# fraunhoferhhi/vvenc

Hardware: AMD Instinct MI355X
Metric: frames/sec + bit-exact vs CPU, 1080p/4K 10-bit preset=faster at 1/2/4/8 GPU (higher is better)
Workload: dtype i16; 1 GPU; BASELINE configs[1]: hot-path work lists RECORDED from the reference encoder (1920x1080 10-bit synthetic clip, 65 frames, preset faster; one picture per temporal layer), replayed resident in HBM: a step = one picture's integer-ME SAD windows + sub-pel SATD stages + table calls + fused TU transform/quant lists + DMVR lists on 5 HIP streams; steps follow the GOP's 1:1:2:4:8:16 layer mix from the key; hip_streams=5, sample_pairs_per_frame=175309451, coefficients_per_frame=6951461, recorded_calls_outside_the_lists=0

## Files before the change

### include/vvenc_hip.h

```cpp
#ifndef VVENC_HIP_H
#define VVENC_HIP_H

#include <stddef.h>
#include <stdint.h>

#ifdef __cplusplus
extern "C" {
#endif

#define VVHIP_API __attribute__((visibility("default")))

enum {
  VVHIP_OK           = 0,
  VVHIP_E_ARG        = -1,
  VVHIP_E_HIP        = -2,
  VVHIP_E_NOMEM      = -3,
  VVHIP_E_UNSUPPORTED= -4
};

typedef struct vvhip_ctx vvhip_ctx;

VVHIP_API int         vvhip_create( vvhip_ctx** out, int device );
VVHIP_API void        vvhip_destroy( vvhip_ctx* ctx );
VVHIP_API const char* vvhip_last_error( const vvhip_ctx* ctx );
// ... 61 lines not shown
VVHIP_API int vvhip_planes_derive( vvhip_ctx* ctx, const int16_t* d_org_base, int org_stride, int org_rows, int16_t* d_org_tiled,
                                   const int16_t* d_cur_base, int cur_stride, int cur_rows, int16_t* d_cur_tiled, int16_t* d_cur_shift1 );
VVHIP_API size_t vvhip_tiled8_elems( int stride, int rows );
VVHIP_API int vvhip_plane_tile8( vvhip_ctx* ctx, const int16_t* d_base, int stride, int rows, int16_t* d_tiled );
VVHIP_API int vvhip_dist_multi_func_tiled( vvhip_ctx* ctx, const int16_t* d_org, int org_stride, const int16_t* d_cur, int cur_stride, const vvhip_tiled_planes* tiled_host, int bit_depth,
                                           const vvhip_dist_fjob* jobs_host, int n_jobs );

VVHIP_API int vvhip_sad_x5_batch( vvhip_ctx* ctx,
                                  const int16_t* d_org, int org_stride,
                                  const int16_t* d_cur, int cur_stride,
                                  int width, int height, int sub_shift, int calc_centre,
                                  const vvhip_dist_item* d_items, int n, uint64_t* d_out5 );

VVHIP_API int vvhip_sad_mask_batch( vvhip_ctx* ctx,
                                    const int16_t* d_org, int org_stride,
                                    const int16_t* d_cur, int cur_stride,
                                    const int16_t* d_mask, int mask_stride, int step_x, int mask_stride2,
                                    int width, int height, int sub_shift, int bit_depth,
                                    const vvhip_dist_item* d_items, const int32_t* d_mask_off, int n, uint64_t* d_out );

VVHIP_API int vvhip_fix_weighted_sse_batch( vvhip_ctx* ctx,
                                            const int16_t* d_org, int org_stride,
                                            const int16_t* d_cur, int cur_stride,
                                            int width, int height, int bit_depth,
                                            const vvhip_dist_item* d_items, const uint32_t* d_weights, int n, uint64_t* d_out );

VVHIP_API int vvhip_sad_surface( vvhip_ctx* ctx,
                                 const int16_t* d_org, int org_stride,
                                 const int16_t* d_ref, int ref_stride,
                                 int width, int height, int sub_shift,
                                 int range_x, int range_y,
                                 const int32_t* d_block_org_off, const int32_t* d_block_ref_off, int n_blocks,
                                 uint32_t* d_out );

enum { VVHIP_DCT2 = 0, VVHIP_DCT8 = 1, VVHIP_DST7 = 2 };

VVHIP_API int vvhip_fwd_transform_batch( vvhip_ctx* ctx, const int16_t* d_resi, int resi_stride, const int32_t* d_resi_off,
                                         int n, int width, int height, int tr_hor, int tr_ver, int bit_depth,
                                         int32_t* d_coef );
VVHIP_API int vvhip_inv_transform_batch( vvhip_ctx* ctx, const int32_t* d_coef,
                                         int n, int width, int height, int tr_hor, int tr_ver, int bit_depth,
                                         int16_t* d_resi, int resi_stride, const int32_t* d_resi_off );

typedef struct { int16_t qp; int16_t flags; } vvhip_tu_qp;

VVHIP_API int vvhip_quant_batch( vvhip_ctx* ctx, const int32_t* d_coef, int n, int width, int height, int bit_depth,
                                 const vvhip_tu_qp* d_qp, int thr_val,
                                 int16_t* d_level, int32_t* d_delta_u ,
                                 int32_t* d_abs_sum, int32_t* d_last_scan_pos );
VVHIP_API int vvhip_dequant_batch( vvhip_ctx* ctx, const int16_t* d_level, int n, int width, int height, int bit_depth,
                                   const vvhip_tu_qp* d_qp, int32_t* d_coef );
VVHIP_API int vvhip_need_rdoq_batch( vvhip_ctx* ctx, const int32_t* d_coef, int n, int width, int height, int bit_depth,
                                     const vvhip_tu_qp* d_qp, uint8_t* d_need );

VVHIP_API int vvhip_dequant_core( vvhip_ctx* ctx, int max_x, int max_y, int scale, const int16_t* d_level, size_t level_stride, int32_t* d_coef,
                                  int right_shift, int input_maximum, int32_t transform_maximum );
VVHIP_API int vvhip_quant_core( vvhip_ctx* ctx, const int32_t* d_coef, int width, int height, int quant_coeff, int q_bits, int64_t add, int thr_val,
                                int16_t* d_level , int32_t* d_delta_u , int32_t* d_abs_sum, int32_t* d_last_scan_pos );
VVHIP_API int vvhip_quant_core_lfnst( vvhip_ctx* ctx, const int32_t* d_coef, int width, int height, int quant_coeff, int q_bits, int64_t add, int thr_val, int lfnst_idx,
                                      int16_t* d_level , int32_t* d_delta_u , int32_t* d_abs_sum, int32_t* d_last_scan_pos );
VVHIP_API int vvhip_need_rdoq_core( vvhip_ctx* ctx, const int32_t* d_coef, size_t num_coeff, int quant_coeff, int64_t offset, int shift, uint8_t* d_need );

typedef struct { int32_t abs_sum; int32_t last_scan_pos; int32_t need_rdoq; int32_t pad; uint64_t sse; } vvhip_tu_stats;

VVHIP_API int vvhip_tu_rdo_batch( vvhip_ctx* ctx, const int16_t* d_resi, int resi_stride, const int32_t* d_resi_off,
                                  int n, int width, int height, int tr_hor, int tr_ver, int bit_depth,
                                  const vvhip_tu_qp* d_qp, int thr_val,
                                  int16_t* d_level, int16_t* d_rec_resi , vvhip_tu_stats* d_stats );

typedef struct
{
  int32_t width, height, tr_hor, tr_ver, n, thr_val;
  const int32_t*     d_resi_off;
  const vvhip_tu_qp* d_qp;
  int16_t*           d_level;
  int16_t*           d_rec_resi;
  vvhip_tu_stats*    d_stats;
} vvhip_tu_job;
VVHIP_API int vvhip_tu_rdo_multi( vvhip_ctx* ctx, const int16_t* d_resi, int resi_stride, int bit_depth, const vvhip_tu_job* jobs_host, int n_jobs );
VVHIP_API int vvhip_tu_rdo_multi_strided( vvhip_ctx* ctx, const int16_t* d_resi, const int32_t* resi_strides_host, int bit_depth, const vvhip_tu_job* jobs_host, int n_jobs );

VVHIP_API int vvhip_tu_set_sparse_outputs( vvhip_ctx* ctx, int on );

VVHIP_API int vvhip_fast_fwd_core( vvhip_ctx* ctx, int tr_size, const int16_t* d_tc, const int32_t* d_src, int32_t* d_dst,
                                   unsigned line, unsigned reduced_line, unsigned cutoff, int shift );
VVHIP_API int vvhip_fast_inv_core( vvhip_ctx* ctx, int tr_size, const int16_t* d_it, const int32_t* d_src, int32_t* d_dst,
                                   unsigned lines, unsigned reduced_lines, unsigned rows );
VVHIP_API int vvhip_round_clip( vvhip_ctx* ctx, int32_t* d_dst, unsigned width, unsigned height, unsigned stride,
                                int32_t out_min, int32_t out_max, int32_t round, int32_t shift );
VVHIP_API int vvhip_cpy_resi( vvhip_ctx* ctx, const int32_t* d_src, int16_t* d_dst, ptrdiff_t stride, unsigned width, unsigned height );
VVHIP_API int vvhip_cpy_coeff( vvhip_ctx* ctx, const int16_t* d_src, ptrdiff_t stride, int32_t* d_dst, unsigned width, unsigned height );

VVHIP_API int vvhip_if_filter( vvhip_ctx* ctx, int taps, int is_vertical, int is_first, int is_last, int bit_depth,
                               const int16_t* d_src, int src_stride, int16_t* d_dst, int dst_stride, int width, int height,
                               const int16_t* coeff_host );
VVHIP_API int vvhip_if_copy( vvhip_ctx* ctx, int is_first, int is_last, int bit_depth,
                             const int16_t* d_src, int src_stride, int16_t* d_dst, int dst_stride, int width, int height, int bi_mc_for_dmvr );

typedef struct { int32_t org_off, ref_off; int16_t frac_x, frac_y; } vvhip_subpel_item;

VVHIP_API int vvhip_interp_luma_batch( vvhip_ctx* ctx, const int16_t* d_ref, int ref_stride, const vvhip_subpel_item* d_items, int n,
                                       int width, int height, int bit_depth, int rnd_res, int filter_mode, int use_alt_hpel,
                                       int16_t* d_out );

VVHIP_API int vvhip_subpel_dist_batch( vvhip_ctx* ctx, int func, const int16_t* d_org, int org_stride, const int16_t* d_ref, int ref_stride,
                                       int width, int height, int bit_depth, int filter_mode, int use_alt_hpel,
                                       const vvhip_subpel_item* d_items, int n, uint64_t* d_out );

VVHIP_API int vvhip_subpel_refine_batch( vvhip_ctx* ctx, int func, const int16_t* d_org, int org_stride, const int16_t* d_ref, int ref_stride,
                                         int width, int height, int bit_depth, int filter_mode, int use_alt_hpel,
                                         const vvhip_subpel_item* d_bases, int n_blocks, const int16_t* offsets_host, int n_offsets, uint64_t* d_out );

typedef struct { const int16_t* d_base; int32_t stride; int32_t reserved; } vvhip_me_plane;
typedef struct { int32_t org_off, ref_off; int16_t width, height; uint8_t org_plane, ref_plane, sub_shift, reserved; int16_t min_dx, min_dy, win_w, win_h; int32_t first_cand, n_cand; } vvhip_me_int_job;
typedef struct { int16_t dx, dy; } vvhip_me_cand;
typedef struct { int32_t org_off, ref_off; int16_t width, height; uint8_t org_plane, ref_plane, i_frac, filter_mode, alt_hpel, func; int8_t base_qx, base_qy; uint16_t mask; uint16_t reserved; } vvhip_me_stage_job;
typedef struct { int32_t org_off, cur_off; uint8_t org_plane, cur_plane, func, sub_shift; int16_t width, height; } vvhip_me_item;
typedef struct { int32_t org_off, cur_off, mask_off; uint8_t org_plane, cur_plane, mask_plane, sub_shift; int16_t width, height; int32_t reserved; } vvhip_me_mask_item;
typedef struct
{
  const vvhip_me_int_job* int_jobs; int32_t n_int_jobs; const vvhip_me_cand* cands; int32_t n_cands;
  const vvhip_me_stage_job* stage_jobs; int32_t n_stage_jobs; const vvhip_me_item* items; int32_t n_items;
  const vvhip_me_mask_item* mask_items; int32_t n_mask_items;
} vvhip_me_lists;
typedef struct vvhip_me_plan vvhip_me_plan;
VVHIP_API int  vvhip_me_plan_create( vvhip_ctx* ctx, const vvhip_me_int_job* int_jobs, int n_int_jobs, const vvhip_me_cand* cands, int n_cands,
                                     const vvhip_me_stage_job* stage_jobs, int n_stage_jobs, const vvhip_me_item* items, int n_items,
                                     int bit_depth, int max_window, vvhip_me_plan** out );
VVHIP_API int  vvhip_me_plan_create_lists( vvhip_ctx* ctx, const vvhip_me_lists* lists, int bit_depth, int max_window, vvhip_me_plan** out );
VVHIP_API void vvhip_me_plan_destroy( vvhip_ctx* ctx, vvhip_me_plan* plan );
VVHIP_API int  vvhip_me_plan_run( vvhip_ctx* ctx, const vvhip_me_plan* plan, const vvhip_me_plane* planes_host, int n_planes,
                                  uint64_t* d_cand_cost, uint64_t* d_stage_cost, uint64_t* d_item_cost );
VVHIP_API int  vvhip_me_plan_run_parts( vvhip_ctx* ctx, const vvhip_me_plan* plan, const vvhip_me_plane* planes_host, int n_planes,
                                        uint64_t* d_cand_cost, uint64_t* d_stage_cost, uint64_t* d_item_cost, int parts );
VVHIP_API int  vvhip_me_plan_set_timing( vvhip_ctx* ctx, vvhip_me_plan* plan, int on );
VVHIP_API int  vvhip_me_plan_last_times( vvhip_ctx* ctx, const vvhip_me_plan* plan, float* ms4_host );
VVHIP_API int  vvhip_me_plan_info( const vvhip_me_plan* plan, int* waves_int, int* waves_stage, int* waves_item, int* lds_bytes );

typedef struct
{
  int32_t dst_off;
  int32_t org_off;
  int32_t ref_off[2];
  int16_t frac[2][2];
  int16_t width, height;
  int8_t  ref_plane[2];
  uint8_t chroma;
  uint8_t alt_hpel;
} vvhip_pred_item;
VVHIP_API int vvhip_pred_inter_batch( vvhip_ctx* ctx, const vvhip_me_plane* planes_host, int n_planes ,
                                      const vvhip_pred_item* items_host, int n, int bit_depth,
                                      int16_t* d_pred, int pred_stride,
                                      const int16_t* d_org , int org_stride, int16_t* d_resi  );
#define VVHIP_PRED_EXT_BDOF     1
#define VVHIP_PRED_EXT_DMVR_PAD 2
typedef struct
{
  uint8_t flags;
  int8_t  pad_dx[2];
  int8_t  pad_dy[2];
  uint8_t rsv[3];
} vvhip_pred_ext;
VVHIP_API int vvhip_pred_inter_batch_ex( vvhip_ctx* ctx, const vvhip_me_plane* planes_host, int n_planes, const vvhip_pred_item* items_host,
                                         const vvhip_pred_ext* ext_host , int n, int bit_depth,
                                         int16_t* d_pred, int pred_stride,
                                         const int16_t* d_org , int org_stride, int16_t* d_resi  );
// ... 108 lines not shown
```

### vvenc_amd/csrc/common.h

```cpp
#pragma once
#include <hip/hip_runtime.h>
#include <stdint.h>
#include <stdio.h>
#include <string>
#include <vector>
#include "../../include/vvenc_hip.h"

struct vvhip_ctx
{
  int          device     = 0;
  hipStream_t  stream     = nullptr;
  hipStream_t  ownStream  = nullptr;
  std::string  lastError;

  int16_t*     d_trMat    = nullptr;
  uint16_t*    d_scan     = nullptr;
  struct VvhipTuMxOps* d_tuMx = nullptr;
  struct VvhipTuMx64Ops* d_tuMx64 = nullptr;
  uint16_t*    d_tuMxPos  = nullptr;
  void*        d_scratch  = nullptr;
  size_t       scratchBytes = 0;
  bool         mctfTiming = false;
  std::vector<hipEvent_t> mctfEv;
  std::vector<int> mctfEvTag;
  unsigned long long* d_mctfStats = nullptr;
  void*        d_subpel   = nullptr;
  size_t       subpelBytes = 0;
  void*        d_tuGen    = nullptr;
  size_t       tuGenBytes = 0;
  std::vector<unsigned char> tuGenLast;
  bool         tuSparse   = false;
  hipStream_t  tuGenStream = nullptr;
  hipEvent_t   tuGenEvent  = nullptr;
  bool         tuGenEventRecorded = false;
  struct PredSched
  {
    void*        d_sched   = nullptr;
    size_t       bytes     = 0;
    std::vector<unsigned char> key, blob;
    size_t       offSubs   = 0, offUnits = 0, offBlend = 0;
    int          units     = 0, ldsPerWave = 0;
    int          unitsEx   = 0, ldsPerWaveEx = 0;
    int          unitsBlend = 0, ldsPerWaveBlend = 0;
    hipStream_t  stream    = nullptr;
    hipEvent_t   event     = nullptr;
    bool         eventRecorded = false;
  } predSched[2];
  void*        d_affSched = nullptr;
  size_t       affBytes   = 0;
  std::vector<unsigned char> affKey, affBlob;
  size_t       affOffSubs = 0, affOffUnits = 0;
  int          affUnits   = 0;
  hipStream_t  affStream  = nullptr;
  hipEvent_t   affEvent   = nullptr;
  bool         affEventRecorded = false;
  bool         blockingSync = false;
  hipEvent_t   syncEvent  = nullptr;
};

inline hipError_t vvhip_wait_stream( vvhip_ctx* ctx )
{
  if( !ctx->blockingSync ) return hipStreamSynchronize( ctx->stream );
  if( !ctx->syncEvent ) return hipErrorInvalidHandle;
  const hipError_t e = hipEventRecord( ctx->syncEvent, ctx->stream );
  return e != hipSuccess ? e : hipEventSynchronize( ctx->syncEvent );
}

int vvhip_fail( vvhip_ctx* ctx, int code, const char* fmt, ... );

#define VVHIP_CHECK_HIP( ctx, expr )                                                        \
  do { hipError_t e_ = ( expr );                                                            \
       if( e_ != hipSuccess ) return vvhip_fail( ctx, VVHIP_E_HIP, "%s: %s (%s:%d)", #expr, \
                                                 hipGetErrorString( e_ ), __FILE__, __LINE__ ); } while( 0 )

#define VVHIP_LAUNCH_CHECK( ctx ) VVHIP_CHECK_HIP( ctx, hipGetLastError() )

static inline __host__ __device__ int trMatOffset( int trType, int log2N )
{
  return trType * 5460 + ( ( 1 << ( 2 * log2N ) ) - 4 ) / 3;
}
static const int kTrMatTotal = 3 * 5460;

static inline __host__ __device__ int scanOffset( int log2w, int log2h )
{
  return ( ( 1 << log2w ) - 1 ) * 127 + ( 1 << log2w ) * ( ( 1 << log2h ) - 1 );
}
static const int kScanTotal = 127 * 127;

static inline __host__ __device__ int mxHw( int h, int s ) { return 8 * ( s >> 2 ) + 4 * h + ( s & 3 ); }
static inline __host__ __device__ int mxSigma( int i )     { return 16 * ( ( i >> 2 ) & 1 ) + 4 * ( i >> 3 ) + ( i & 3 ); }
struct VvhipTuMxOps
{
  int8_t  nat[64][16];
  int8_t  rowP[64][16];
  int8_t  natT[64][16];
  int8_t  colP[64][16];
  int32_t rowSum[32];
  int32_t colSum[32];
};

struct VvhipTuMx64Ops
{
  int8_t  natX[2][64][16];
  int8_t  rowPY[2][64][16];
  int8_t  natTY[2][64][16];
  int8_t  colPX[2][64][16];
  int32_t rowSum[32];
  int32_t colSum[64];
  uint16_t pos[64][16];
};

void vvhip_build_tr_matrix( int trType, int log2N, int16_t* out );
void vvhip_build_scan_order( int log2w, int log2h, uint32_t* out );
void vvhip_cg_size( int log2w, int log2h, int* log2CGw, int* log2CGh );
// ... 61 lines not shown
```

### vvenc_amd/csrc/ctx.hip

```cpp
#include "common.h"
#include <stdarg.h>
#include <stdlib.h>
#include <string.h>
#include <memory>
#include <atomic>
#include <vector>

static std::string g_createError;

int vvhip_fail( vvhip_ctx* ctx, int code, const char* fmt, ... )
{
  char buf[512];
  va_list ap;
  va_start( ap, fmt );
  vsnprintf( buf, sizeof( buf ), fmt, ap );
  va_end( ap );
  if( ctx ) ctx->lastError = buf; else g_createError = buf;
  return code;
}

static const int16_t kDct2Cos[65] = {
  64, 91, 90, 90, 90, 90, 90, 90, 89, 88, 88, 87, 87, 86, 85, 84, 83, 83, 82, 81, 80, 79, 78, 77, 75, 73, 73, 71, 70, 69, 67, 65, 64,
  62, 61, 59, 57, 56, 54, 52, 50, 48, 46, 44, 43, 41, 38, 37, 36, 33, 31, 28, 25, 24, 22, 20, 18, 15, 13, 11, 9, 7, 4, 2, 0 };
static const int16_t kDst7Sin4[4]   = { 29, 55, 74, 84 };
// ... 126 lines not shown
  {
    const int l2 = 2 + z, n = 1 << l2;
    for( int t = 0; t < 3; t++ )
    {
      const int16_t* m = mats.data() + trMatOffset( t, l2 );
      auto big = [&]( int r, int c ) -> int { return ( r / n == c / n ) ? m[( r % n ) * n + ( c % n )] : 0; };
      VvhipTuMxOps& o = mx[t * 4 + z];
      for( int r = 0; r < 32; r++ )
      {
        int rs = 0, cs = 0;
        for( int c = 0; c < 32; c++ )
        {
          if( big( r, c ) < -128 || big( r, c ) > 127 ) return vvhip_fail( nullptr, VVHIP_E_HIP, "vvhip_create: transform matrix entry outside 8 bits" );
          rs += big( r, c ); cs += big( c, r );
        }
        o.rowSum[r] = 128 * rs; o.colSum[r] = 128 * cs;
      }
      for( int l = 0; l < 64; l++ )
        for( int k = 0; k < 16; k++ )
        {
          const int h = l / 32, r = l % 32;
          o.nat[l][k]  = ( int8_t ) big( r, 16 * h + k );
          o.rowP[l][k] = ( int8_t ) big( mxSigma( r ), mxHw( h, k ) );
          o.natT[l][k] = ( int8_t ) big( 16 * h + k, r );
          o.colP[l][k] = ( int8_t ) big( mxHw( h, k ), mxSigma( r ) );
        }
    }
    const uint16_t* sc = scans.data() + scanOffset( l2, l2 );
    std::vector<uint16_t> inv( n * n );
    for( int i = 0; i < n * n; i++ ) inv[sc[i]] = ( uint16_t ) i;
    for( int l = 0; l < 64; l++ )
      for( int v = 0; v < 16; v++ ) mxPos[( z * 64 + l ) * 16 + v] = inv[( ( 16 * ( l / 32 ) + v ) % n ) * n + ( l % 32 ) % n];
  }
  {
    std::unique_ptr<VvhipTuMx64Ops> o64p( new VvhipTuMx64Ops );
    VvhipTuMx64Ops& o64 = *o64p;
    const int16_t* m = mats.data() + trMatOffset( VVHIP_DCT2, 6 );
    auto T = [&]( int r, int c ) -> int { return m[r * 64 + c]; };
    for( int r = 0; r < 32; r++ ) { int rs = 0; for( int c = 0; c < 64; c++ ) { if( T( r, c ) < -128 || T( r, c ) > 127 ) return vvhip_fail( nullptr, VVHIP_E_HIP, "vvhip_create: 64-point matrix entry outside 8 bits" ); rs += T( r, c ); } o64.rowSum[r] = 128 * rs; }
    for( int c = 0; c < 64; c++ ) { int cs = 0; for( int r = 0; r < 32; r++ ) cs += T( r, c ); o64.colSum[c] = 128 * cs; }
    for( int q = 0; q < 2; q++ )
      for( int l = 0; l < 64; l++ )
        for( int k = 0; k < 16; k++ )
        {
          const int h = l / 32, r = l % 32;
          o64.natX[q][l][k]  = ( int8_t ) T( r, 32 * q + 16 * h + k );
          o64.rowPY[q][l][k] = ( int8_t ) T( mxSigma( r ), 32 * q + mxHw( h, k ) );
          o64.natTY[q][l][k] = ( int8_t ) T( 16 * h + k, 32 * q + r );
          o64.colPX[q][l][k] = ( int8_t ) T( mxHw( h, k ), 32 * q + mxSigma( r ) );
        }
    const uint16_t* sc = scans.data() + scanOffset( 6, 6 );
    std::vector<uint16_t> inv( 64 * 64, 0xffff );
    for( int i = 0; i < 32 * 32; i++ ) inv[sc[i]] = ( uint16_t ) i;
    for( int l = 0; l < 64; l++ ) for( int v = 0; v < 16; v++ ) o64.pos[l][v] = inv[( 16 * ( l / 32 ) + v ) * 64 + l % 32];
    VVHIP_CHECK_HIP( nullptr, hipMalloc( ( void** ) &ctx->d_tuMx64, sizeof( o64 ) ) );
    VVHIP_CHECK_HIP( nullptr, hipMemcpy( ctx->d_tuMx64, &o64, sizeof( o64 ), hipMemcpyHostToDevice ) );
  }
  VVHIP_CHECK_HIP( nullptr, hipMalloc( ( void** ) &ctx->d_tuMx, mx.size() * sizeof( VvhipTuMxOps ) ) );
  VVHIP_CHECK_HIP( nullptr, hipMalloc( ( void** ) &ctx->d_tuMxPos, mxPos.size() * sizeof( uint16_t ) ) );
  VVHIP_CHECK_HIP( nullptr, hipMemcpy( ctx->d_tuMx, mx.data(), mx.size() * sizeof( VvhipTuMxOps ), hipMemcpyHostToDevice ) );
  VVHIP_CHECK_HIP( nullptr, hipMemcpy( ctx->d_tuMxPos, mxPos.data(), mxPos.size() * sizeof( uint16_t ), hipMemcpyHostToDevice ) );
  VVHIP_CHECK_HIP( nullptr, hipMalloc( ( void** ) &ctx->d_trMat, mats.size() * sizeof( int16_t ) ) );
  VVHIP_CHECK_HIP( nullptr, hipMalloc( ( void** ) &ctx->d_scan, scans.size() * sizeof( uint16_t ) ) );
  VVHIP_CHECK_HIP( nullptr, hipMemcpy( ctx->d_trMat, mats.data(), mats.size() * sizeof( int16_t ), hipMemcpyHostToDevice ) );
  VVHIP_CHECK_HIP( nullptr, hipMemcpy( ctx->d_scan, scans.data(), scans.size() * sizeof( uint16_t ), hipMemcpyHostToDevice ) );
  guard.c = nullptr;
  *out = ctx;
  return VVHIP_OK;
}

void vvhip_destroy( vvhip_ctx* ctx )
{
  if( !ctx ) return;
  ( void ) hipSetDevice( ctx->device );
  if( ctx->ownStream ) ( void ) hipStreamSynchronize( ctx->ownStream );
  if( ctx->d_trMat ) ( void ) hipFree( ctx->d_trMat );
  if( ctx->d_scan ) ( void ) hipFree( ctx->d_scan );
  if( ctx->d_tuMx ) ( void ) hipFree( ctx->d_tuMx );
  if( ctx->d_tuMxPos ) ( void ) hipFree( ctx->d_tuMxPos );
  if( ctx->d_tuMx64 ) ( void ) hipFree( ctx->d_tuMx64 );
  if( ctx->d_scratch ) ( void ) hipFree( ctx->d_scratch );
  if( ctx->d_subpel ) ( void ) hipFree( ctx->d_subpel );
  if( ctx->d_tuGen ) ( void ) hipFree( ctx->d_tuGen );
  if( ctx->syncEvent ) ( void ) hipEventDestroy( ctx->syncEvent );
  if( ctx->tuGenEvent ) ( void ) hipEventDestroy( ctx->tuGenEvent );
  for( vvhip_ctx::PredSched& S : ctx->predSched )
  {
    if( S.d_sched ) ( void ) hipFree( S.d_sched );
    if( S.event ) ( void ) hipEventDestroy( S.event );
  }
  if( ctx->d_affSched ) ( void ) hipFree( ctx->d_affSched );
  if( ctx->affEvent ) ( void ) hipEventDestroy( ctx->affEvent );
  if( ctx->d_mctfStats ) ( void ) hipFree( ctx->d_mctfStats );
  for( hipEvent_t e : ctx->mctfEv ) ( void ) hipEventDestroy( e );
  if( ctx->ownStream ) ( void ) hipStreamDestroy( ctx->ownStream );
  delete ctx;
}

const char* vvhip_last_error( const vvhip_ctx* ctx ) { return ctx ? ctx->lastError.c_str() : g_createError.c_str(); }

int vvhip_set_stream( vvhip_ctx* ctx, void* hip_stream )
{
  if( !ctx ) return VVHIP_E_ARG;
  if( hip_stream )
  {
    hipDevice_t dev = 0;
    if( hipStreamGetDevice( ( hipStream_t ) hip_stream, &dev ) == hipSuccess && ( int ) dev != ctx->device )
      return vvhip_fail( ctx, VVHIP_E_ARG, "vvhip_set_stream: the stream belongs to device %d, the context to device %d", ( int ) dev, ctx->device );
    ( void ) hipGetLastError();
  }
  ctx->stream = ( hipStream_t ) hip_stream;
  return VVHIP_OK;
}

int vvhip_use_own_stream( vvhip_ctx* ctx )
{
  if( !ctx ) return VVHIP_E_ARG;
  ctx->stream = ctx->ownStream;
  return VVHIP_OK;
}

void* vvhip_get_stream( vvhip_ctx* ctx ) { return ctx ? ( void* ) ctx->stream : nullptr; }

int vvhip_set_blocking_sync( vvhip_ctx* ctx, int on )
{
  if( !ctx ) return VVHIP_E_ARG;
  ctx->blockingSync = on != 0;
  return VVHIP_OK;
}

int vvhip_sync( vvhip_ctx* ctx )
{
  if( !ctx ) return VVHIP_E_ARG;
  VVHIP_CHECK_HIP( ctx, vvhip_wait_stream( ctx ) );
  return VVHIP_OK;
}

int vvhip_sync_all_devices( vvhip_ctx* ctx )
{
  if( !ctx ) return VVHIP_E_ARG;
  int prev = 0, n = 0;
  VVHIP_CHECK_HIP( ctx, hipGetDevice( &prev ) );
  VVHIP_CHECK_HIP( ctx, hipGetDeviceCount( &n ) );
  const uint64_t live = g_liveDevices.load();
  hipError_t first = hipSuccess;
  for( int d = 0; d < n && d < 64; d++ )
  {
    if( !( ( live >> d ) & 1 ) ) continue;
    hipError_t e = hipSetDevice( d );
    if( e == hipSuccess ) e = hipDeviceSynchronize();
    if( e != hipSuccess && first == hipSuccess ) first = e;
  }
  ( void ) hipSetDevice( prev );
  VVHIP_CHECK_HIP( ctx, first );
  return VVHIP_OK;
}

struct vvhip_graph { hipGraph_t graph; hipGraphExec_t exec; };

int vvhip_graph_begin( vvhip_ctx* ctx )
{
  if( !ctx ) return VVHIP_E_ARG;
  VVHIP_CHECK_HIP( ctx, hipStreamBeginCapture( ctx->stream, hipStreamCaptureModeThreadLocal ) );
  return VVHIP_OK;
}

// ... 185 lines not shown
```

### vvenc_amd/csrc/trquant.hip

```cpp
#include "common.h"
#include <stdlib.h>
#include <string.h>
#include <algorithm>
#include <vector>

namespace {

typedef uint32_t u32x2 __attribute__( ( ext_vector_type( 2 ) ) );
typedef uint32_t u32x4 __attribute__( ( ext_vector_type( 4 ) ) );
typedef short    s16x2 __attribute__( ( ext_vector_type( 2 ) ) );

__device__ __forceinline__ int clip3i( int lo, int hi, int v ) { return v < lo ? lo : ( v > hi ? hi : v ); }
__device__ __forceinline__ int sat16( int v ) { return clip3i( -32768, 32767, v ); }
__device__ __forceinline__ int dot2( uint32_t a, uint32_t b, int acc )
{
  return __builtin_amdgcn_sdot2( __builtin_bit_cast( s16x2, a ), __builtin_bit_cast( s16x2, b ), acc, false );
}

struct TrGeom
{
  int w, h, log2w, log2h;
  int skipW, skipH;
  int shift1, shift2;
};
// ... 708 lines not shown
      for( int jj = 0; jj < NO; jj++ )
      {
        const int j = o0 + jj;
        int acc;
        DOT_ROW( acc, dqp, &sMat[3][j * N] );
        tile[j * P + cidx] = ( int16_t ) ( colLive ? sat16( ( int ) ( ( uint32_t ) acc + ( uint32_t ) rnd1 ) >> gi.shift1 ) : 0 );
      }
    }
    WAVE_SYNC();
    if( A.phaseLimit == 7 ) return;
    unsigned long long sse = 0;
    {
      uint32_t t[ND];
  #pragma unroll
      for( int c = 0; c < NC; c++ ) { const u32x4 v = *reinterpret_cast<const u32x4*>( &tile[r * P + 8 * c] ); t[4 * c] = v.x; t[4 * c + 1] = v.y; t[4 * c + 2] = v.z; t[4 * c + 3] = v.w; }
      const int rnd2 = 1 << ( gi.shift2 - 1 );
      for( int c8 = 0; c8 < NOC; c8++ )
      {
        u32x4 xv = { 0, 0, 0, 0 };
        if( valid ) xv = reinterpret_cast<const U16*>( src + o0 + 8 * c8 )->v;
        const uint32_t xs[4] = { xv.x, xv.y, xv.z, xv.w };
        uint32_t rp[4];
  #pragma unroll
        for( int pr = 0; pr < 4; pr++ )
        {
          int rv[2];
  #pragma unroll
          for( int e = 0; e < 2; e++ )
          {
            int acc;
            DOT_ROW( acc, t, &sMat[2][( o0 + 8 * c8 + 2 * pr + e ) * N] );
            rv[e] = sat16( ( int ) ( ( uint32_t ) acc + ( uint32_t ) rnd2 ) >> gi.shift2 );
          }
          rp[pr] = ( uint32_t ) ( rv[0] & 0xffff ) | ( ( uint32_t ) rv[1] << 16 );
          const int d0 = ( int ) ( int16_t ) ( xs[pr] & 0xffff ) - rv[0], d1 = ( ( int ) xs[pr] >> 16 ) - rv[1];
          sse += ( unsigned long long ) ( ( long long ) d0 * d0 ) + ( unsigned long long ) ( ( long long ) d1 * d1 );
        }
        if( rec && valid )
        {
          u32x4 v; v.x = rp[0]; v.y = rp[1]; v.z = rp[2]; v.w = rp[3];
          *reinterpret_cast<u32x4*>( rec + ( size_t ) tu * N * N + r * N + o0 + 8 * c8 ) = v;
        }
      }
    }
  #undef DOT_ROW
  #undef WAVE_SYNC
    sse = vvhipGroupSum64( sse, LPT, lane );
    if( stats && valid && li == 0 )
    {
      vvhip_tu_stats st; st.abs_sum = ( int32_t ) absSum; st.last_scan_pos = ( int32_t ) last; st.need_rdoq = ( int32_t ) need; st.pad = 0; st.sse = sse;
      stats[tu] = st;
    }
  }
}

template<int N, int SPLIT>
__global__ void __launch_bounds__( 256 )
tuRdoRowKernel( const int16_t* __restrict__ resi, int resiStride, TuRowArgs args )
{
  __shared__ __attribute__( ( aligned( 16 ) ) ) unsigned char smem[TuRowLds<N, SPLIT>::bytes];
  tuRdoRowBody<N, SPLIT>( smem, blockIdx.x, resi, resiStride, args );
}

struct TuMultiJobs { int nJobs; int blockStart[4]; int size[4]; TuRowArgs j[4]; };

__global__ void __launch_bounds__( 256 )
tuRdoRowMultiKernel( const int16_t* __restrict__ resi, int resiStride, TuMultiJobs jobs )
{
  constexpr int B32 = TuRowLds<32, 2>::bytes, B16 = TuRowLds<16, 2>::bytes, B8 = TuRowLds<8, 1>::bytes;
  __shared__ __attribute__( ( aligned( 16 ) ) ) unsigned char smem[B32 > B16 ? ( B32 > B8 ? B32 : B8 ) : ( B16 > B8 ? B16 : B8 )];
  int k = 0;
#pragma unroll
  for( int i = 1; i < 4; i++ ) if( i < jobs.nJobs && ( int ) blockIdx.x >= jobs.blockStart[i] ) k = i;
  const int blk = blockIdx.x - jobs.blockStart[k];
  if( jobs.size[k] == 32 )      tuRdoRowBody<32, 2>( smem, blk, resi, resiStride, jobs.j[k] );
  else if( jobs.size[k] == 16 ) tuRdoRowBody<16, 2>( smem, blk, resi, resiStride, jobs.j[k] );
  else                          tuRdoRowBody<8, 1>( smem, blk, resi, resiStride, jobs.j[k] );
}


#ifndef TUMX_ZERO_MIN_N
#define TUMX_ZERO_MIN_N 8
#endif
typedef int v4i  __attribute__( ( ext_vector_type( 4 ) ) );
typedef int v16i __attribute__( ( ext_vector_type( 16 ) ) );

struct TuMxArgs
{
  const int32_t* resiOff; int n;
  int shF1, shF2, shI1, shI2, skipW, skipH;
  QGeom q;
  const VvhipTuMxOps* opH; const VvhipTuMxOps* opV; const uint16_t* pos;
  const vvhip_tu_qp* qps; int thrVal;
  int16_t* level; int16_t* rec; vvhip_tu_stats* stats;
  int tiles;
  int phaseLimit;
  int waveStride;
  int resiStride;
};

__device__ __forceinline__ void mxSplit( const int* d, v4i& lo, v4i& hi )
{
#pragma unroll
  for( int g = 0; g < 4; g++ )
  {
    const uint32_t p01 = __builtin_amdgcn_perm( ( uint32_t ) d[4 * g + 1], ( uint32_t ) d[4 * g], 0x05040100u );
    const uint32_t p23 = __builtin_amdgcn_perm( ( uint32_t ) d[4 * g + 3], ( uint32_t ) d[4 * g + 2], 0x05040100u );
    lo[g] = ( int ) ( __builtin_amdgcn_perm( p23, p01, 0x06040200u ) ^ 0x80808080u );
    hi[g] = ( int ) __builtin_amdgcn_perm( p23, p01, 0x07050301u );
  }
}

typedef unsigned short u16x2v __attribute__( ( ext_vector_type( 2 ) ) );
__device__ __forceinline__ uint32_t pkMaxU16( uint32_t a, uint32_t b )
{
  return __builtin_bit_cast( uint32_t, __builtin_elementwise_max( __builtin_bit_cast( u16x2v, a ), __builtin_bit_cast( u16x2v, b ) ) );
}
__device__ __forceinline__ uint32_t tuMxGroupMaxPk16( uint32_t v, int G, int lane )
{
  v = pkMaxU16( v, ( uint32_t ) VVHIP_DPP( v, VVHIP_DPP_XOR1 ) );
  v = pkMaxU16( v, ( uint32_t ) VVHIP_DPP( v, VVHIP_DPP_XOR2 ) );
  if( G >= 8 ) v = pkMaxU16( v, ( uint32_t ) VVHIP_DPP( v, VVHIP_DPP_HALF_MIRROR ) );
  if( G >= 16 ) v = pkMaxU16( v, ( uint32_t ) VVHIP_DPP( v, VVHIP_DPP_MIRROR ) );
  if( G >= 32 )
  {
    const uint32_t r0 = ( uint32_t ) __builtin_amdgcn_readlane( ( int ) v, 0 ),  r1 = ( uint32_t ) __builtin_amdgcn_readlane( ( int ) v, 16 );
    const uint32_t r2 = ( uint32_t ) __builtin_amdgcn_readlane( ( int ) v, 32 ), r3 = ( uint32_t ) __builtin_amdgcn_readlane( ( int ) v, 48 );
    const uint32_t a = pkMaxU16( r0, r1 ), b = pkMaxU16( r2, r3 );
    v = G == 64 ? pkMaxU16( a, b ) : ( lane < 32 ? a : b );
  }
  return v;
}

__device__ __forceinline__ uint32_t sadU32( uint32_t a, uint32_t b, uint32_t acc ) { uint32_t r; asm( "v_sad_u32 %0, %1, %2, %3" : "=v"( r ) : "v"( a ), "v"( b ), "v"( acc ) ); return r; }
__device__ __forceinline__ int med3i( int x, int lo, int hi ) { int r; asm( "v_med3_i32 %0, %1, %2, %3" : "=v"( r ) : "v"( x ), "v"( lo ), "v"( hi ) ); return r; }

struct TuMxQ { int scale, qBits, thres, iscale, rightShift, inMax; long long addQ, addN; };
__device__ __forceinline__ int tuMxSel6( int r, int a0, int a1, int a2, int a3, int a4, int a5 )
{
  return r == 0 ? a0 : r == 1 ? a1 : r == 2 ? a2 : r == 3 ? a3 : r == 4 ? a4 : a5;
}
__device__ __forceinline__ TuMxQ tuMxParams( const QGeom& q, const vvhip_tu_qp qq, const int thrVal )
{
  TuMxQ P;
  const int per = qq.qp / 6, rem = qq.qp - 6 * per;
  const int trShift = 15 - q.bitDepth - q.log2w;
  P.scale = tuMxSel6( rem, 26214, 23302, 20560, 18396, 16384, 14564 );
  P.iscale = tuMxSel6( rem, 40, 45, 51, 57, 64, 72 );
  P.qBits = 14 + per + trShift;
  P.addQ = ( long long ) ( ( qq.flags & 1 ) ? 171 : 85 ) << ( P.qBits - 9 );
  P.addN = ( long long ) ( ( qq.flags & 2 ) ? 171 : 256 ) << ( P.qBits - 9 );
  P.thres = P.qBits ? ( int32_t ) ( ( int64_t ) thrVal << ( P.qBits - 1 ) ) : ( int32_t ) ( ( int64_t ) ( thrVal >> 1 ) << P.qBits );
  P.rightShift = 6 - ( trShift + per );
  int tgt = 32 + P.rightShift - 7; if( tgt > 16 ) tgt = 16;
  P.inMax = ( 1 << ( tgt - 1 ) ) - 1;
  return P;
}

typedef short s16x2v __attribute__( ( ext_vector_type( 2 ) ) );
__device__ __forceinline__ void mxSplitSat( const int* d, v4i& lo, v4i& hi )
{
#pragma unroll
  for( int g = 0; g < 4; g++ )
  {
    const uint32_t p01 = __builtin_bit_cast( uint32_t, __builtin_amdgcn_cvt_pk_i16( d[4 * g], d[4 * g + 1] ) );
    const uint32_t p23 = __builtin_bit_cast( uint32_t, __builtin_amdgcn_cvt_pk_i16( d[4 * g + 2], d[4 * g + 3] ) );
    lo[g] = ( int ) ( __builtin_amdgcn_perm( p23, p01, 0x06040200u ) ^ 0x80808080u );
    hi[g] = ( int ) __builtin_amdgcn_perm( p23, p01, 0x07050301u );
  }
}

template<int N>
__device__ __forceinline__ void
tuMxBody( int16_t* __restrict__ stage, int32_t* __restrict__ sInit, v4i* __restrict__ sOps, const int waveIndex, const int16_t* __restrict__ resi, const int resiStride, const TuMxArgs& A )
{
  constexpr int TPS = 32 / N, TPT = TPS * TPS, R = N >= 16 ? 1 : 16 / N, VPR = 16 / R, G = N == 32 ? 64 : N;
  constexpr int PS = N < 8 ? N : 8, NP = 16 / PS;
  constexpr int LP = 40;
  struct __attribute__( ( packed, aligned( 2 ) ) ) U16 { u32x4 v; };
  struct __attribute__( ( packed, aligned( 2 ) ) ) U8 { u32x2 v; };
  const int lane = threadIdx.x & 63, h = lane >> 5, c32 = lane & 31;
  const int blkL = c32 / N, inL = c32 % N;
  const int blk0 = ( 16 * h ) / N;
  const v16i zero16 = { 0, 0, 0, 0, 0, 0, 0, 0, 0, 0, 0, 0, 0, 0, 0, 0 };
#define WAVE_SYNC() { __builtin_amdgcn_fence( __ATOMIC_ACQ_REL, "wavefront" ); __builtin_amdgcn_wave_barrier(); }
#define MX_PASS( HA, HB, LA, LB, C, SH ) { v16i acc_ = __builtin_amdgcn_mfma_i32_32x32x32_i8( HA, HB, zero16, 0, 0, 0 );                      \
    _Pragma( "unroll" ) for( int v = 0; v < 16; v++ ) acc_[v] = ( acc_[v] << 8 ) + C[v];                                                     \
    acc_ = __builtin_amdgcn_mfma_i32_32x32x32_i8( LA, LB, acc_, 0, 0, 0 );                                                                   \
    _Pragma( "unroll" ) for( int v = 0; v < 16; v++ ) d[v] = acc_[v] >> ( SH ); }
#define TUMX_KEEP( ARR ) { int k_ = 0; _Pragma( "unroll" ) for( int v = 0; v < 16; v++ ) k_ ^= ARR[v]; if( k_ == 0x12345678 ) A.stats[0].pad = 1; }

  auto loadResidual = [&]( const int tile, uint32_t* xr )
  {
#pragma unroll
    for( int c = 0; c < NP; c++ )
    {
      const int X0 = 16 * h + PS * c;
      const int tu = tile * TPT + blkL * TPS + X0 / N;
      const bool ok = tile < A.tiles && tu < A.n;
      const int16_t* src = resi + ( ok ? A.resiOff[tu] : 0 ) + ( ptrdiff_t ) inL * resiStride + X0 % N;
      if( PS == 8 )
      {
        u32x4 v = { 0, 0, 0, 0 };
        if( ok ) v = reinterpret_cast<const U16*>( src )->v;
        xr[4 * c] = v.x; xr[( 4 * c + 1 ) & 7] = v.y; xr[( 4 * c + 2 ) & 7] = v.z; xr[( 4 * c + 3 ) & 7] = v.w;
      }
      else
      {
        u32x2 v = { 0, 0 };
        if( ok ) v = reinterpret_cast<const U8*>( src )->v;
        xr[( 2 * c ) & 7] = v.x; xr[( 2 * c + 1 ) & 7] = v.y;
      }
    }
  };
  uint32_t xr[8];
  loadResidual( waveIndex, xr );

  const int rndF1 = A.shF1 > 0 ? 1 << ( A.shF1 - 1 ) : 0, rndF2 = 1 << ( A.shF2 - 1 ), rndI1 = 1 << ( A.shI1 - 1 ), rndI2 = 1 << ( A.shI2 - 1 );
  const bool liveCol = inL < N - A.skipW, liveRow = mxSigma( c32 ) % N < N - A.skipH;
  const v4i zero4 = { 0, 0, 0, 0 };
  sOps[lane]       = liveCol ? *reinterpret_cast<const v4i*>( A.opH->nat[lane] ) : zero4;
  sOps[64 + lane]  = liveRow ? *reinterpret_cast<const v4i*>( A.opV->rowP[lane] ) : zero4;
  const int cP1 = ( liveCol ? A.opH->rowSum[c32] : 0 ) + rndF1, cI1 = A.opV->colSum[c32] + rndI1;
  sInit[c32]      = ( c32 % N < N - A.skipH ? A.opV->rowSum[c32] : 0 ) + rndF2;
  sInit[32 + c32] = A.opH->colSum[c32] + rndI2;
  uint32_t pos[16];
  {
    const u32x4 p0 = *reinterpret_cast<const u32x4*>( A.pos + lane * 16 ), p1 = *reinterpret_cast<const u32x4*>( A.pos + lane * 16 + 8 );
    const uint32_t pw[8] = { p0.x, p0.y, p0.z, p0.w, p1.x, p1.y, p1.z, p1.w };
#pragma unroll
    for( int v = 0; v < 16; v++ ) pos[v] = ( v & 1 ) ? pw[v >> 1] >> 16 : pw[v >> 1] & 0xffffu;
  }
  WAVE_SYNC();
  if( ( A.phaseLimit & 0xff ) == 1 ) return;

  for( int tile = waveIndex; tile < A.tiles; tile += A.waveStride )
  {
    v4i aLo, aHi;
    if( tile != waveIndex ) loadResidual( tile, xr );
#pragma unroll
    for( int g = 0; g < 4; g++ )
    {
      aLo[g] = ( int ) ( __builtin_amdgcn_perm( xr[2 * g + 1], xr[2 * g], 0x06040200u ) ^ 0x80808080u );
      aHi[g] = ( int ) __builtin_amdgcn_perm( xr[2 * g + 1], xr[2 * g], 0x07050301u );
    }
    int eng[R];
    bool smallResi = false;
    if( N >= TUMX_ZERO_MIN_N )
    {
      typedef unsigned short u16x2e __attribute__( ( ext_vector_type( 2 ) ) );
      uint32_t magn = 0;
#pragma unroll
      for( int r = 0; r < R; r++ ) eng[r] = 0;
#pragma unroll
      for( int k = 0; k < 8; k++ )
      {
        const int slot = ( PS * ( k / ( PS / 2 ) ) ) / N < R ? ( PS * ( k / ( PS / 2 ) ) ) / N : 0;
        eng[slot] = dot2( xr[k], xr[k], eng[slot] );
        magn |= __builtin_bit_cast( uint32_t, __builtin_bit_cast( u16x2e, xr[k] ) + __builtin_bit_cast( u16x2e, 0x10001000u ) ) & 0xe000e000u;
      }
      smallResi = __builtin_amdgcn_ballot_w64( magn != 0 ) == 0ull;
    }
    vvhip_tu_qp qqs[R];
#pragma unroll
    for( int r = 0; r < R; r++ ) { const int tu = tile * TPT + ( blk0 + r ) * TPS + blkL; qqs[r] = tu < A.n ? A.qps[tu] : vvhip_tu_qp{ 32, 0 }; }
    if( ( A.phaseLimit & 0xff ) == 2 ) { int k_ = 0; _Pragma( "unroll" ) for( int g = 0; g < 4; g++ ) k_ ^= aLo[g] ^ aHi[g]; if( k_ == 0x12345678 ) A.stats[0].pad = 1; continue; }

    int d[16];
    v4i bLo, bHi;
    {
      v16i c;
#pragma unroll
      for( int v = 0; v < 16; v++ ) c[v] = cP1;
      const v4i opP1 = sOps[lane];
      MX_PASS( aHi, opP1, aLo, opP1, c, A.shF1 );
      mxSplitSat( d, bLo, bHi );
    }
    {
      v16i c;
#pragma unroll
      for( int g = 0; g < 4; g++ ) { const v4i t = *reinterpret_cast<const v4i*>( &sInit[h * 16 + 4 * g] ); c[4 * g] = t.x; c[4 * g + 1] = t.y; c[4 * g + 2] = t.z; c[4 * g + 3] = t.w; }
      const v4i opP2 = sOps[64 + lane];
      MX_PASS( opP2, bHi, opP2, bLo, c, A.shF2 );
    }
    if( ( A.phaseLimit & 0xff ) == 3 ) { TUMX_KEEP( d ); continue; }

    uint32_t last[R], need[R], big[R];
    bool wide = false, someLevel = false;
#pragma unroll
    for( int r = 0; r < R; r++ )
    {
      const TuMxQ P = tuMxParams( A.q, qqs[r], A.thrVal );
      uint32_t l = 0, mx = 0, bg = 0;
      const int thr4 = P.thres >> 2;
#pragma unroll
      for( int v = r * VPR; v < ( r + 1 ) * VPR; v++ )
      {
        const uint32_t ac = ( uint32_t ) abs( d[v] );
        mx = ac > mx ? ac : mx;
        l = ( ac != 0 && pos[v] > l ) ? pos[v] : l;
        bg = ( ( int ) __umul24( ac, ( uint32_t ) P.scale ) > thr4 && pos[v] > bg ) ? pos[v] : bg;
      }
      { const uint32_t lb = tuMxGroupMaxPk16( l | ( bg << 16 ), G, lane ); l = lb & 0xffffu; bg = lb >> 16; }
      mx = vvhipGroupMax32( mx, G, lane );
      need[r] = ( uint32_t ) ( ( int32_t ) ( ( ( int64_t ) mx * P.scale + P.addN ) >> P.qBits ) != 0 );
      someLevel |= ( ( ( int64_t ) mx * P.scale + P.addQ ) >> P.qBits ) != 0;
      wide |= mx >= 65536u || P.qBits > 30 || P.qBits < 9;
      last[r] = l; big[r] = bg;
    }
    const bool narrow = __builtin_amdgcn_ballot_w64( wide ) == 0ull;
    if( !narrow )
#pragma unroll
      for( int r = 0; r < R; r++ )
      {
        const TuMxQ P = tuMxParams( A.q, qqs[r], A.thrVal );
        uint32_t bg = 0;
#pragma unroll
        for( int v = r * VPR; v < ( r + 1 ) * VPR; v++ )
          bg = ( ( long long ) abs( d[v] ) * ( P.scale << 2 ) > ( long long ) P.thres && pos[v] > bg ) ? pos[v] : bg;
        big[r] = vvhipGroupMax32( bg, G, lane );
      }
#pragma unroll
    for( int r = 0; r < R; r++ )
      if( last[r] >= 16 )
      {
        if( big[r] < 16 ) last[r] = 15;
        else if( ( big[r] >> 4 ) != ( last[r] >> 4 ) ) last[r] = ( big[r] >> 4 ) * 16 + 15;
      }
    if( ( A.phaseLimit & 0xff ) == 4 ) { TUMX_KEEP( d ); continue; }
    typedef unsigned short u16x2t __attribute__( ( ext_vector_type( 2 ) ) );
#define TUMX_TAIL( STORE_REC ) { \
    unsigned long long sse[R]; \
_Pragma( "unroll" ) \
    for( int r = 0; r < R; r++ ) sse[r] = 0; \
    uint32_t rpAll[8]; \
    uint32_t magn = 0; \
_Pragma( "unroll" ) \
    for( int k = 0; k < 8; k++ ) \
    { \
      rpAll[k] = __builtin_bit_cast( uint32_t, __builtin_amdgcn_cvt_pk_i16( d[2 * k], d[2 * k + 1] ) ); \
      magn |= __builtin_bit_cast( uint32_t, __builtin_bit_cast( u16x2t, rpAll[k] ) + __builtin_bit_cast( u16x2t, 0x10001000u ) ) & 0xe000e000u; \
      magn |= __builtin_bit_cast( uint32_t, __builtin_bit_cast( u16x2t, xr2[k] ) + __builtin_bit_cast( u16x2t, 0x10001000u ) ) & 0xe000e000u; \
    } \
    const bool smallDiff = __builtin_amdgcn_ballot_w64( magn != 0 ) == 0ull; \
    uint32_t sse32[R]; \
_Pragma( "unroll" ) \
    for( int r = 0; r < R; r++ ) sse32[r] = 0; \
_Pragma( "unroll" ) \
    for( int c = 0; c < NP; c++ ) \
    { \
      const int X0 = 16 * h + PS * c; \
      const int tu = tile * TPT + blkL * TPS + X0 / N; \
      uint32_t rp[PS / 2]; \
_Pragma( "unroll" ) \
      for( int k = 0; k < PS / 2; k++ ) \
      { \
        const int xi = ( PS / 2 ) * c + k; \
        rp[k] = rpAll[xi]; \
        const int slot = ( PS * c ) / N < R ? ( PS * c ) / N : 0; \
        if( smallDiff ) \
        { \
          const uint32_t df = __builtin_bit_cast( uint32_t, __builtin_bit_cast( s16x2, xr2[xi] ) - __builtin_bit_cast( s16x2, rp[k] ) ); \
          sse32[slot] = ( uint32_t ) dot2( df, df, ( int ) sse32[slot] ); \
        } \
        else \
        { \
          const int e0 = ( int ) ( int16_t ) ( xr2[xi] & 0xffff ) - ( int ) ( int16_t ) ( rp[k] & 0xffff ), e1 = ( ( int ) xr2[xi] >> 16 ) - ( ( int ) rp[k] >> 16 ); \
          sse[slot] += ( unsigned long long ) ( ( long long ) e0 * e0 ) + ( unsigned long long ) ( ( long long ) e1 * e1 ); \
        } \
      } \
      if( ( STORE_REC ) && A.rec && tu < A.n ) \
      { \
        int16_t* dst = A.rec + ( size_t ) tu * N * N + inL * N + X0 % N; \
        if( PS == 8 ) { u32x4 v; v.x = rp[0]; v.y = rp[1 % ( PS / 2 )]; v.z = rp[2 % ( PS / 2 )]; v.w = rp[3 % ( PS / 2 )]; *reinterpret_cast<u32x4*>( dst ) = v; } \
        else          { u32x2 v; v.x = rp[0]; v.y = rp[1 % ( PS / 2 )]; *reinterpret_cast<u32x2*>( dst ) = v; } \
      } \
    } \
_Pragma( "unroll" ) \
    for( int r = 0; r < R; r++ ) \
    { \
      const unsigned long long t = vvhipGroupSum64( smallDiff ? ( unsigned long long ) sse32[r] : sse[r], G, lane ); \
      const int tu = tile * TPT + blkL * TPS + blk0 + r; \
      if( A.stats && ( N < 32 || h == 0 ) && inL == r && tu < A.n ) A.stats[tu].sse = t; \
    } }
    const bool allZero = ( N >= TUMX_ZERO_MIN_N ) && __builtin_amdgcn_ballot_w64( someLevel ) == 0ull;
    uint32_t xr2[8];
#define TUMX_REREAD() { _Pragma( "unroll" ) for( int c = 0; c < NP; c++ )                                                                \
      {                                                                                                                                 \
        const int X0 = 16 * h + PS * c;                                                                                                 \
        const int tu = tile * TPT + blkL * TPS + X0 / N;                                                                                \
        const int16_t* src = resi + ( tu < A.n ? A.resiOff[tu] : 0 ) + ( ptrdiff_t ) inL * resiStride + X0 % N;                         \
        if( PS == 8 )                                                                                                                   \
        {                                                                                                                               \
          u32x4 v = { 0, 0, 0, 0 };                                                                                                     \
          if( tu < A.n ) v = reinterpret_cast<const U16*>( src )->v;                                                                    \
          xr2[4 * c] = v.x; xr2[( 4 * c + 1 ) & 7] = v.y; xr2[( 4 * c + 2 ) & 7] = v.z; xr2[( 4 * c + 3 ) & 7] = v.w;                   \
        }                                                                                                                               \
        else                                                                                                                            \
        {                                                                                                                               \
          u32x2 v = { 0, 0 };                                                                                                           \
          if( tu < A.n ) v = reinterpret_cast<const U8*>( src )->v;                                                                     \
          xr2[( 2 * c ) & 7] = v.x; xr2[( 2 * c + 1 ) & 7] = v.y;                                                                       \
        }                                                                                                                               \
      } }
    if( allZero )
    {
#pragma unroll
      for( int r = 0; r < R; r++ )
      {
        const int tu = tile * TPT + ( blk0 + r ) * TPS + blkL;
        if( A.stats && ( N < 32 || h == 0 ) && inL == r && tu < A.n )
        {
          int32_t* st = reinterpret_cast<int32_t*>( A.stats + tu );
          st[0] = 0; st[1] = ( int32_t ) last[r]; st[2] = ( int32_t ) need[r]; st[3] = 0;
        }
      }
      if( !( A.phaseLimit & 0x100 ) )
#pragma unroll
      for( int u = 0; u < 16 / PS; u++ )
      {
        const int q = lane + 64 * u, Y = q / ( 32 / PS ), X = PS * ( q % ( 32 / PS ) );
        const int tu = tile * TPT + ( Y / N ) * TPS + X / N;
        if( tu < A.n )
        {
          const size_t at = ( size_t ) tu * N * N + ( Y % N ) * N + X % N;
          if( PS == 8 ) { if( A.level ) *reinterpret_cast<u32x4*>( A.level + at ) = u32x4{ 0, 0, 0, 0 }; if( A.rec ) *reinterpret_cast<u32x4*>( A.rec + at ) = u32x4{ 0, 0, 0, 0 }; }
          else          { if( A.level ) *reinterpret_cast<u32x2*>( A.level + at ) = u32x2{ 0, 0 }; if( A.rec ) *reinterpret_cast<u32x2*>( A.rec + at ) = u32x2{ 0, 0 }; }
        }
      }
      if( smallResi )
      {
#pragma unroll
        for( int r = 0; r < R; r++ )
        {
          const unsigned long long t = vvhipGroupSum64( ( unsigned long long ) ( uint32_t ) eng[r], G, lane );
          const int tu = tile * TPT + blkL * TPS + blk0 + r;
          if( A.stats && ( N < 32 || h == 0 ) && inL == r && tu < A.n ) A.stats[tu].sse = t;
        }
        continue;
      }
      TUMX_REREAD()
#pragma unroll
      for( int v = 0; v < 16; v++ ) d[v] = 0;
      TUMX_TAIL( false )
      continue;
    }
    uint32_t absSum[R];
#define TUMX_LEVELS( MEXPR )                                                                                                           \
    _Pragma( "unroll" ) for( int r = 0; r < R; r++ )                                                                                   \
    {                                                                                                                                  \
      const TuMxQ P = tuMxParams( A.q, qqs[r], A.thrVal );                                                                             \
      uint32_t sum = 0;                                                                                                                \
      const int rsPos = P.rightShift > 0 ? P.rightShift : 0, rndDq = P.rightShift > 0 ? 1 << ( P.rightShift - 1 ) : 0;                \
      const int iscaleL = P.rightShift < 0 ? P.iscale << ( -P.rightShift ) : P.iscale;                                                 \
      _Pragma( "unroll" ) for( int v = r * VPR; v < ( r + 1 ) * VPR; v++ )                                                             \
      {                                                                                                                                \
        const int cv = d[v];                                                                                                           \
        const uint32_t ac = ( uint32_t ) abs( cv );                                                                                    \
        uint32_t m = MEXPR;                                                                                                            \
        m = pos[v] <= last[r] ? m : 0u;                                                                                                \
        sum += m;                                                                                                                      \
        const int sm = cv < 0 ? -( int32_t ) m : ( int32_t ) m;                                                                        \
        const int lv = clip3i( -32768, 32767, sm );                                                                                    \
        stage[( 16 * h + v ) * LP + c32] = ( int16_t ) lv;                                                                             \
        const int cl = med3i( lv, ~P.inMax, P.inMax );                                                                                 \
        const int32_t w_ = ( int32_t ) ( ( uint32_t ) __mul24( cl, iscaleL ) + ( uint32_t ) rndDq ) >> rsPos;    \
        d[v] = clip3i( -32768, 32767, w_ );                                                                                            \
      }                                                                                                                                \
      absSum[r] = sum;                                                                                                                 \
    }
    if( narrow )
    {
#pragma unroll
      for( int r = 0; r < R; r++ )
      {
        const TuMxQ P = tuMxParams( A.q, qqs[r], A.thrVal );
        uint32_t sum = 0;
        const int addP = ( int ) P.addQ, addM = ( int ) ( ( 1u << P.qBits ) - 1u ) - addP;
        const int rsPos = P.rightShift > 0 ? P.rightShift : 0, rndDq = P.rightShift > 0 ? 1 << ( P.rightShift - 1 ) : 0;
        const int iscaleL = P.rightShift < 0 ? P.iscale << ( -P.rightShift ) : P.iscale;
#pragma unroll
        for( int v = r * VPR; v < ( r + 1 ) * VPR; v++ )
        {
          const int cv = d[v];
          int sm = ( __mul24( cv, P.scale ) + ( cv < 0 ? addM : addP ) ) >> P.qBits;
          sm = pos[v] <= last[r] ? sm : 0;
          sum = sadU32( ( uint32_t ) ( sm + ( 1 << 24 ) ), 1u << 24, sum );
          const int lv = clip3i( -32768, 32767, sm );
          stage[( 16 * h + v ) * LP + c32] = ( int16_t ) lv;
          const int cl = med3i( lv, ~P.inMax, P.inMax );
          const int32_t w_ = ( int32_t ) ( ( uint32_t ) __mul24( cl, iscaleL ) + ( uint32_t ) rndDq ) >> rsPos;
          d[v] = clip3i( -32768, 32767, w_ );
        }
        absSum[r] = sum;
      }
    }
    else { TUMX_LEVELS( ( uint32_t ) ( int32_t ) ( ( ( int64_t ) ac * P.scale + P.addQ ) >> P.qBits ) ) }
#undef TUMX_LEVELS
#pragma unroll
    for( int r = 0; r < R; r++ )
    {
      const uint32_t sum = vvhipGroupSum32( absSum[r], G, lane );
      const int tu = tile * TPT + ( blk0 + r ) * TPS + blkL;
      if( A.stats && ( N < 32 || h == 0 ) && inL == r && tu < A.n )
      {
        int32_t* st = reinterpret_cast<int32_t*>( A.stats + tu );
        st[0] = ( int32_t ) sum; st[1] = ( int32_t ) last[r]; st[2] = ( int32_t ) need[r]; st[3] = 0;
      }
    }
    if( ( A.phaseLimit & 0xff ) == 5 ) { TUMX_KEEP( d ); continue; }
    WAVE_SYNC();
    if( A.level )
#pragma unroll
      for( int u = 0; u < 16 / PS; u++ )
      {
        const int q = lane + 64 * u, Y = q / ( 32 / PS ), X = PS * ( q % ( 32 / PS ) );
        const int tu = tile * TPT + ( Y / N ) * TPS + X / N;
        if( tu < A.n )
        {
          int16_t* dst = A.level + ( size_t ) tu * N * N + ( Y % N ) * N + X % N;
          if( PS == 8 ) *reinterpret_cast<u32x4*>( dst ) = *reinterpret_cast<const u32x4*>( &stage[Y * LP + X] );
          else          *reinterpret_cast<u32x2*>( dst ) = *reinterpret_cast<const u32x2*>( &stage[Y * LP + X] );
        }
      }
    WAVE_SYNC();

    if( ( A.phaseLimit & 0xff ) == 6 ) { TUMX_KEEP( d ); continue; }
    mxSplit( d, aLo, aHi );
    {
      v16i c;
#pragma unroll
      for( int v = 0; v < 16; v++ ) c[v] = cI1;
      const v4i opI1 = *reinterpret_cast<const v4i*>( A.opV->natT[lane] );
      MX_PASS( aHi, opI1, aLo, opI1, c, A.shI1 );
      mxSplitSat( d, bLo, bHi );
    }
    TUMX_REREAD()
    {
      v16i c;
#pragma unroll
      for( int g = 0; g < 4; g++ ) { const v4i t = *reinterpret_cast<const v4i*>( &sInit[32 + h * 16 + 4 * g] ); c[4 * g] = t.x; c[4 * g + 1] = t.y; c[4 * g + 2] = t.z; c[4 * g + 3] = t.w; }
      const v4i opI2 = *reinterpret_cast<const v4i*>( A.opH->colP[lane] );
      MX_PASS( opI2, bHi, opI2, bLo, c, A.shI2 );
    }
    if( ( A.phaseLimit & 0xff ) == 7 ) { TUMX_KEEP( d ); continue; }
    TUMX_TAIL( true )
  }
#undef WAVE_SYNC
#undef TUMX_KEEP
#undef MX_PASS
#undef TUMX_REREAD
#undef TUMX_TAIL
}

__device__ __forceinline__ void
tuMx64Body( int16_t* __restrict__ stage, int32_t* __restrict__ sInit , v4i* __restrict__ sOps , const int waveIndex,
            const int16_t* __restrict__ resi, const int resiStride, const TuMxArgs& A )
{
  constexpr int LP = 40;
  struct __attribute__( ( packed, aligned( 2 ) ) ) U16 { u32x4 v; };
  const VvhipTuMx64Ops* __restrict__ O = reinterpret_cast<const VvhipTuMx64Ops*>( A.opH );
  const int lane = threadIdx.x & 63, h = lane >> 5, c32 = lane & 31;
  const v16i zero16 = { 0, 0, 0, 0, 0, 0, 0, 0, 0, 0, 0, 0, 0, 0, 0, 0 };
#define WAVE_SYNC() { __builtin_amdgcn_fence( __ATOMIC_ACQ_REL, "wavefront" ); __builtin_amdgcn_wave_barrier(); }
  const int rndF1 = 1 << ( A.shF1 - 1 ), rndF2 = 1 << ( A.shF2 - 1 ), rndI1 = 1 << ( A.shI1 - 1 ), rndI2 = 1 << ( A.shI2 - 1 );
#pragma unroll
  for( int q = 0; q < 2; q++ )
  {
    sOps[( 0 + q ) * 64 + lane] = *reinterpret_cast<const v4i*>( O->natX[q][lane] );
    sOps[( 2 + q ) * 64 + lane] = *reinterpret_cast<const v4i*>( O->rowPY[q][lane] );
  }
  const int cP1 = O->rowSum[c32] + rndF1;
  const int cI1[2] = { O->colSum[c32] + rndI1, O->colSum[32 + c32] + rndI1 };
  sInit[c32] = O->rowSum[c32] + rndF2;
  sInit[32 + lane] = O->colSum[lane] + rndI2;
  uint32_t pos[16];
  {
    const u32x4 p0 = *reinterpret_cast<const u32x4*>( &O->pos[lane][0] ), p1 = *reinterpret_cast<const u32x4*>( &O->pos[lane][8] );
    const uint32_t pw[8] = { p0.x, p0.y, p0.z, p0.w, p1.x, p1.y, p1.z, p1.w };
#pragma unroll
    for( int v = 0; v < 16; v++ ) pos[v] = ( v & 1 ) ? pw[v >> 1] >> 16 : pw[v >> 1] & 0xffffu;
  }
  WAVE_SYNC();

  for( int tu = waveIndex; tu < A.n; tu += A.waveStride )
  {
    const int16_t* src = resi + A.resiOff[tu];
    const vvhip_tu_qp qq = A.qps[tu];
    int d[16];
    v4i bLo[2], bHi[2];
    typedef unsigned short u16x2z __attribute__( ( ext_vector_type( 2 ) ) );
    int eng = 0;
    uint32_t magn = 0;
#pragma unroll
    for( int t = 0; t < 2; t++ )
    {
      v16i acc = zero16;
      v4i aLo[2];
#pragma unroll
      for( int c = 0; c < 2; c++ )
      {
        const int16_t* p = src + ( ptrdiff_t ) ( 32 * t + c32 ) * resiStride + 32 * c + 16 * h;
        const u32x4 x0 = reinterpret_cast<const U16*>( p )->v, x1 = reinterpret_cast<const U16*>( p + 8 )->v;
        const uint32_t xr[8] = { x0.x, x0.y, x0.z, x0.w, x1.x, x1.y, x1.z, x1.w };
        v4i aHi;
#pragma unroll
        for( int g = 0; g < 4; g++ )
        {
          aLo[c][g] = ( int ) ( __builtin_amdgcn_perm( xr[2 * g + 1], xr[2 * g], 0x06040200u ) ^ 0x80808080u );
          aHi[g] = ( int ) __builtin_amdgcn_perm( xr[2 * g + 1], xr[2 * g], 0x07050301u );
        }
#pragma unroll
        for( int k = 0; k < 8; k++ )
        {
          eng = dot2( xr[k], xr[k], eng );
          magn |= __builtin_bit_cast( uint32_t, __builtin_bit_cast( u16x2z, xr[k] ) + __builtin_bit_cast( u16x2z, 0x10001000u ) ) & 0xe000e000u;
        }
        acc = __builtin_amdgcn_mfma_i32_32x32x32_i8( aHi, sOps[c * 64 + lane], acc, 0, 0, 0 );
      }
#pragma unroll
      for( int v = 0; v < 16; v++ ) acc[v] = ( acc[v] << 8 ) + cP1;
#pragma unroll
      for( int c = 0; c < 2; c++ ) acc = __builtin_amdgcn_mfma_i32_32x32x32_i8( aLo[c], sOps[c * 64 + lane], acc, 0, 0, 0 );
#pragma unroll
      for( int v = 0; v < 16; v++ ) d[v] = acc[v] >> A.shF1;
      mxSplitSat( d, bLo[t], bHi[t] );
    }
    {
      v16i acc = zero16;
#pragma unroll
      for( int t = 0; t < 2; t++ ) acc = __builtin_amdgcn_mfma_i32_32x32x32_i8( sOps[( 2 + t ) * 64 + lane], bHi[t], acc, 0, 0, 0 );
#pragma unroll
      for( int g = 0; g < 4; g++ )
      {
        const v4i t4 = *reinterpret_cast<const v4i*>( &sInit[h * 16 + 4 * g] );
        acc[4 * g] = ( acc[4 * g] << 8 ) + t4.x; acc[4 * g + 1] = ( acc[4 * g + 1] << 8 ) + t4.y; acc[4 * g + 2] = ( acc[4 * g + 2] << 8 ) + t4.z; acc[4 * g + 3] = ( acc[4 * g + 3] << 8 ) + t4.w;
      }
#pragma unroll
      for( int t = 0; t < 2; t++ ) acc = __builtin_amdgcn_mfma_i32_32x32x32_i8( sOps[( 2 + t ) * 64 + lane], bLo[t], acc, 0, 0, 0 );
#pragma unroll
      for( int v = 0; v < 16; v++ ) d[v] = acc[v] >> A.shF2;
    }
    const TuMxQ P = tuMxParams( A.q, qq, A.thrVal );
    uint32_t last = 0, mx = 0, big = 0;
    const int thr4 = P.thres >> 2;
#pragma unroll
    for( int v = 0; v < 16; v++ )
    {
      const uint32_t ac = ( uint32_t ) abs( d[v] );
      mx = ac > mx ? ac : mx;
      last = ( ac != 0 && pos[v] > last ) ? pos[v] : last;
      big = ( ( int ) __umul24( ac, ( uint32_t ) P.scale ) > thr4 && pos[v] > big ) ? pos[v] : big;
    }
    { const uint32_t lb = tuMxGroupMaxPk16( last | ( big << 16 ), 64, lane ); last = lb & 0xffffu; big = lb >> 16; }
    mx = vvhipGroupMax32( mx, 64, lane );
    const uint32_t need = ( uint32_t ) ( ( int32_t ) ( ( ( int64_t ) mx * P.scale + P.addN ) >> P.qBits ) != 0 );
    const bool narrow = __builtin_amdgcn_ballot_w64( mx >= 65536u || P.qBits > 30 || P.qBits < 9 ) == 0ull;
    if( !narrow )
    {
      big = 0;
#pragma unroll
      for( int v = 0; v < 16; v++ ) big = ( ( long long ) abs( d[v] ) * ( P.scale << 2 ) > ( long long ) P.thres && pos[v] > big ) ? pos[v] : big;
      big = vvhipGroupMax32( big, 64, lane );
    }
    if( last >= 16 )
    {
      if( big < 16 ) last = 15;
      else if( ( big >> 4 ) != ( last >> 4 ) ) last = ( big >> 4 ) * 16 + 15;
    }
    if( __builtin_amdgcn_ballot_w64( ( ( ( int64_t ) mx * P.scale + P.addQ ) >> P.qBits ) != 0 ) == 0ull )
    {
      if( A.stats && lane == 0 )
      {
        int32_t* st = reinterpret_cast<int32_t*>( A.stats + tu );
        st[0] = 0; st[1] = ( int32_t ) last; st[2] = ( int32_t ) need; st[3] = 0;
      }
      if( !( A.phaseLimit & 0x100 ) )
      {
        char* zr = reinterpret_cast<char*>( A.rec + ( size_t ) tu * 4096 );
        char* zl = reinterpret_cast<char*>( A.level + ( size_t ) tu * 4096 );
        uint32_t zo = ( uint32_t ) lane * 16u;
        asm volatile( "" : "+v"( zo ) );
        const u32x4 z4 = { 0, 0, 0, 0 };
#pragma unroll
        for( int u = 0; u < 8; u++ )
        {
          if( A.rec ) *reinterpret_cast<u32x4*>( zr + ( zo + 1024u * u ) ) = z4;
          if( A.level ) *reinterpret_cast<u32x4*>( zl + ( zo + 1024u * u ) ) = z4;
        }
      }
      unsigned long long sse0 = ( unsigned long long ) ( uint32_t ) eng;
      if( __builtin_amdgcn_ballot_w64( magn != 0 ) != 0ull )
      {
        sse0 = 0;
#pragma nounroll
        for( int tc = 0; tc < 4; tc++ )
        {
          const int t = tc >> 1, c = tc & 1;
          const int16_t* p = src + ( ptrdiff_t ) ( 32 * t + c32 ) * resiStride + 32 * c + 16 * h;
          const u32x4 x0 = reinterpret_cast<const U16*>( p )->v, x1 = reinterpret_cast<const U16*>( p + 8 )->v;
          const uint32_t xr[8] = { x0.x, x0.y, x0.z, x0.w, x1.x, x1.y, x1.z, x1.w };
#pragma unroll
          for( int k = 0; k < 8; k++ )
          {
            const int e0 = ( int ) ( int16_t ) ( xr[k] & 0xffff ), e1 = ( int ) xr[k] >> 16;
            sse0 += ( unsigned long long ) ( ( long long ) e0 * e0 ) + ( unsigned long long ) ( ( long long ) e1 * e1 );
          }
        }
      }
      sse0 = vvhipGroupSum64( sse0, 64, lane );
      if( A.stats && lane == 0 ) A.stats[tu].sse = sse0;
      continue;
    }
    uint32_t sum = 0;
    {
      const int addP = ( int ) P.addQ, addM = ( int ) ( ( 1u << ( P.qBits & 31 ) ) - 1u ) - addP;
      const int rsPos = P.rightShift > 0 ? P.rightShift : 0, rndDq = P.rightShift > 0 ? 1 << ( P.rightShift - 1 ) : 0;
      const int iscaleL = P.rightShift < 0 ? P.iscale << ( -P.rightShift ) : P.iscale;
#define TU64_LEVEL( SMEXPR )                                                                                                         \
      _Pragma( "unroll" ) for( int v = 0; v < 16; v++ )                                                                                 \
      {                                                                                                                                 \
        const int cv = d[v];                                                                                                            \
        int sm = SMEXPR;                                                                                                                \
        sm = pos[v] <= last ? sm : 0;                                                                                                   \
        sum += ( uint32_t ) abs( sm );                                                                                                  \
        const int lv = clip3i( -32768, 32767, sm );                                                                                     \
        stage[( 16 * h + v ) * LP + c32] = ( int16_t ) lv;                                                                              \
        const int cl = med3i( lv, ~P.inMax, P.inMax );                                                                                  \
        const int32_t w_ = ( int32_t ) ( ( uint32_t ) __mul24( cl, iscaleL ) + ( uint32_t ) rndDq ) >> rsPos;                           \
        d[v] = clip3i( -32768, 32767, w_ );                                                                                             \
      }
      if( narrow ) { TU64_LEVEL( ( __mul24( cv, P.scale ) + ( cv < 0 ? addM : addP ) ) >> P.qBits ) }
      else { TU64_LEVEL( ( cv < 0 ? -( int ) ( ( ( int64_t ) abs( cv ) * P.scale + P.addQ ) >> P.qBits ) : ( int ) ( ( ( int64_t ) abs( cv ) * P.scale + P.addQ ) >> P.qBits ) ) ) }
#undef TU64_LEVEL
    }
    sum = vvhipGroupSum32( sum, 64, lane );
    if( A.stats && lane == 0 )
    {
      int32_t* st = reinterpret_cast<int32_t*>( A.stats + tu );
      st[0] = ( int32_t ) sum; st[1] = ( int32_t ) last; st[2] = ( int32_t ) need; st[3] = 0;
    }
    WAVE_SYNC();
    int laneL = lane;
    asm volatile( "" : "+v"( laneL ) );
    const int hL = laneL >> 5, c32L = laneL & 31;
    if( A.level )
#pragma unroll
      for( int u = 0; u < 8; u++ )
      {
        const int q = laneL + 64 * u, Y = q >> 3, X = 8 * ( q & 7 );
        u32x4 v = { 0, 0, 0, 0 };
        if( Y < 32 && X < 32 ) v = *reinterpret_cast<const u32x4*>( &stage[Y * LP + X] );
        *reinterpret_cast<u32x4*>( A.level + ( size_t ) tu * 4096 + Y * 64 + X ) = v;
      }
    WAVE_SYNC();
    v4i aLo, aHi;
    mxSplit( d, aLo, aHi );
#pragma unroll
    for( int t = 0; t < 2; t++ )
    {
      v16i c;
#pragma unroll
      for( int v = 0; v < 16; v++ ) c[v] = cI1[t];
      const v4i op = *reinterpret_cast<const v4i*>( O->natTY[t][laneL] );
      v16i acc = __builtin_amdgcn_mfma_i32_32x32x32_i8( aHi, op, zero16, 0, 0, 0 );
#pragma unroll
      for( int v = 0; v < 16; v++ ) acc[v] = ( acc[v] << 8 ) + c[v];
      acc = __builtin_amdgcn_mfma_i32_32x32x32_i8( aLo, op, acc, 0, 0, 0 );
#pragma unroll
      for( int v = 0; v < 16; v++ ) d[v] = acc[v] >> A.shI1;
      mxSplitSat( d, bLo[t], bHi[t] );
    }
    unsigned long long sse = 0;
#pragma unroll
    for( int c = 0; c < 2; c++ )
#pragma unroll
      for( int t = 0; t < 2; t++ )
      {
        const int16_t* p = src + ( ptrdiff_t ) ( 32 * t + c32 ) * resiStride + 32 * c + 16 * h;
        const u32x4 x0 = reinterpret_cast<const U16*>( p )->v, x1 = reinterpret_cast<const U16*>( p + 8 )->v;
        const uint32_t xr[8] = { x0.x, x0.y, x0.z, x0.w, x1.x, x1.y, x1.z, x1.w };
        v16i ci;
#pragma unroll
        for( int g = 0; g < 4; g++ ) { const v4i t4 = *reinterpret_cast<const v4i*>( &sInit[32 + 32 * c + hL * 16 + 4 * g] ); ci[4 * g] = t4.x; ci[4 * g + 1] = t4.y; ci[4 * g + 2] = t4.z; ci[4 * g + 3] = t4.w; }
        const v4i op = *reinterpret_cast<const v4i*>( O->colPX[c][laneL] );
        v16i acc = __builtin_amdgcn_mfma_i32_32x32x32_i8( op, bHi[t], zero16, 0, 0, 0 );
#pragma unroll
        for( int v = 0; v < 16; v++ ) acc[v] = ( acc[v] << 8 ) + ci[v];
        acc = __builtin_amdgcn_mfma_i32_32x32x32_i8( op, bLo[t], acc, 0, 0, 0 );
        typedef unsigned short u16x2t __attribute__( ( ext_vector_type( 2 ) ) );
        uint32_t rp[8], magn = 0;
#pragma unroll
        for( int k = 0; k < 8; k++ )
        {
// ... 160 lines not shown
        int sm;
        if( narrow ) sm = ( __mul24( cv, P.scale ) + ( cv < 0 ? addM : addP ) ) >> P.qBits;
        else { const int m = ( int ) ( ( ( int64_t ) abs( cv ) * P.scale + P.addQ ) >> P.qBits ); sm = cv < 0 ? -m : m; }
        sm = pos[v] <= last ? sm : 0;
        sum += ( uint32_t ) abs( sm );
        const int lv = clip3i( -32768, 32767, sm );
        stage[( 16 * h + v ) * LP + c32] = ( int16_t ) lv;
        const int cl = med3i( lv, ~P.inMax, P.inMax );
        const int32_t w_ = ( int32_t ) ( ( uint32_t ) __mul24( cl, iscaleL ) + ( uint32_t ) rndDq ) >> rsPos;
        d[v] = clip3i( -32768, 32767, w_ );
      }
    }
    sum = vvhipGroupSum32( sum, 64, lane );
    if( A.stats && p == 0 && lane == 0 )
    {
      int32_t* st = reinterpret_cast<int32_t*>( A.stats + tu );
      st[0] = ( int32_t ) sum; st[1] = ( int32_t ) last; st[2] = ( int32_t ) need; st[3] = 0;
    }
    WAVE_SYNC();
    if( A.level )
#pragma unroll
      for( int u = 0; u < 4; u++ )
      {
        const int q = lane + 64 * ( 4 * p + u ), Y = q >> 3, X = 8 * ( q & 7 );
        u32x4 v = { 0, 0, 0, 0 };
        if( Y < 32 && X < 32 ) v = *reinterpret_cast<const u32x4*>( &stage[Y * LP + X] );
        *reinterpret_cast<u32x4*>( A.level + ( size_t ) tu * 4096 + Y * 64 + X ) = v;
      }
    WAVE_SYNC();
    v4i aLo, aHi;
    mxSplit( d, aLo, aHi );
    {
      v16i c;
#pragma unroll
      for( int v = 0; v < 16; v++ ) c[v] = cI1;
      const v4i op = sOps[4 * 64 + lane];
      const v16i lo = __builtin_amdgcn_mfma_i32_32x32x32_i8( aLo, op, c, 0, 0, 0 );
      const v16i hi = __builtin_amdgcn_mfma_i32_32x32x32_i8( aHi, op, zero16, 0, 0, 0 );
#pragma unroll
      for( int v = 0; v < 16; v++ ) d[v] = ( ( hi[v] << 8 ) + lo[v] ) >> A.shI1;
      mxSplitSat( d, bLo, bHi );
    }
    unsigned long long sse = 0;
#pragma unroll
    for( int c = 0; c < 2; c++ )
    {
      const int16_t* q = src + ( ptrdiff_t ) c32 * resiStride + 32 * c + 16 * h;
      const u32x4 x0 = reinterpret_cast<const U16*>( q )->v, x1 = reinterpret_cast<const U16*>( q + 8 )->v;
      const uint32_t xr[8] = { x0.x, x0.y, x0.z, x0.w, x1.x, x1.y, x1.z, x1.w };
      v16i ci;
#pragma unroll
      for( int g = 0; g < 4; g++ ) { const v4i t4 = *reinterpret_cast<const v4i*>( &sInit[32 + 32 * c + h * 16 + 4 * g] ); ci[4 * g] = t4.x; ci[4 * g + 1] = t4.y; ci[4 * g + 2] = t4.z; ci[4 * g + 3] = t4.w; }
      const v4i op = sOps[( 6 + c ) * 64 + lane];
      const v16i lo = __builtin_amdgcn_mfma_i32_32x32x32_i8( op, bLo, ci, 0, 0, 0 );
      const v16i hi = __builtin_amdgcn_mfma_i32_32x32x32_i8( op, bHi, zero16, 0, 0, 0 );
      uint32_t rp[8];
#pragma unroll
      for( int k = 0; k < 8; k++ )
      {
        const int v0 = ( ( hi[2 * k] << 8 ) + lo[2 * k] ) >> A.shI2, v1 = ( ( hi[2 * k + 1] << 8 ) + lo[2 * k + 1] ) >> A.shI2;
        rp[k] = __builtin_bit_cast( uint32_t, __builtin_amdgcn_cvt_pk_i16( v0, v1 ) );
        const int e0 = ( int ) ( int16_t ) ( xr[k] & 0xffff ) - ( int ) ( int16_t ) ( rp[k] & 0xffff ), e1 = ( ( int ) xr[k] >> 16 ) - ( ( int ) rp[k] >> 16 );
        sse += ( unsigned long long ) ( ( long long ) e0 * e0 ) + ( unsigned long long ) ( ( long long ) e1 * e1 );
      }
      if( A.rec )
      {
        int16_t* dst = A.rec + ( size_t ) tu * 4096 + ( 32 * p + c32 ) * 64 + 32 * c + 16 * h;
        u32x4 a, b; a.x = rp[0]; a.y = rp[1]; a.z = rp[2]; a.w = rp[3]; b.x = rp[4]; b.y = rp[5]; b.z = rp[6]; b.w = rp[7];
        *reinterpret_cast<u32x4*>( dst ) = a; *reinterpret_cast<u32x4*>( dst + 8 ) = b;
      }
    }
    sse = vvhipGroupSum64( sse, 64, lane );
    if( lane == 0 ) { xMine[16] = ( int32_t ) ( uint32_t ) sse; xMine[XP + 16] = ( int32_t ) ( uint32_t ) ( sse >> 32 ); }
    tuMxPairSync( ctr, gen, lane );
    if( A.stats && p == 0 && lane == 0 )
    {
      const unsigned long long o = ( unsigned long long ) ( uint32_t ) xOther[16] | ( ( unsigned long long ) ( uint32_t ) xOther[XP + 16] << 32 );
      A.stats[tu].sse = sse + o;
    }
  }
#undef WAVE_SYNC
}

struct TuMxJobs { int nJobs; int pair64; int waveStart[8]; int size[8]; TuMxArgs j[8]; };

template<int KIND, int WPB>
__global__ void __launch_bounds__( 64 * WPB, KIND == 3 ? 2 : 3 )
tuMxMultiKernel( const int16_t* __restrict__ resi, int resiStride, TuMxJobs jobs )
{
  constexpr bool WITH4 = KIND >= 1, WITH64 = KIND >= 2, PAIR64 = KIND == 3;
  static_assert( WPB == 4 || ( WPB == 1 && !PAIR64 ), "the pair form needs both waves of a pair in one workgroup" );
  __shared__ __attribute__( ( aligned( 16 ) ) ) int16_t stage[WPB][32 * 40];
  __shared__ __attribute__( ( aligned( 16 ) ) ) int32_t sInit[WPB][WITH64 ? 96 : 64];
  __shared__ v4i sOps[WPB][PAIR64 ? 512 : ( WITH64 ? 256 : 128 )];
  __shared__ int32_t xch[PAIR64 ? 2 : 1][PAIR64 ? 2 * 64 * 17 : 1];
  __shared__ uint32_t pairCtr[2];
  if( PAIR64 ) { if( threadIdx.x < 2 ) pairCtr[threadIdx.x] = 0; __syncthreads(); }
  const int wv = WPB == 1 ? 0 : __builtin_amdgcn_readfirstlane( ( int ) ( threadIdx.x >> 6 ) );
  const int wave = blockIdx.x * WPB + wv;
  int k = 0;
#pragma unroll
  for( int i = 1; i < 8; i++ ) if( i < jobs.nJobs && wave >= jobs.waveStart[i] ) k = i;
  const int w = wave - jobs.waveStart[k];
  if( w >= jobs.j[k].waveStride ) return;
  const int rs = jobs.j[k].resiStride ? jobs.j[k].resiStride : resiStride;
  if( jobs.size[k] == 32 )      tuMxBody<32>( stage[wv], sInit[wv], sOps[wv], w, resi, rs, jobs.j[k] );
  else if( jobs.size[k] == 16 ) tuMxBody<16>( stage[wv], sInit[wv], sOps[wv], w, resi, rs, jobs.j[k] );
  else if( jobs.size[k] == 8 )  tuMxBody<8>( stage[wv], sInit[wv], sOps[wv], w, resi, rs, jobs.j[k] );
  else if( WITH4 && jobs.size[k] == 4 )   tuMxBody<4>( stage[wv], sInit[wv], sOps[wv], w, resi, rs, jobs.j[k] );
  else if( WITH64 && jobs.size[k] == 64 )
  {
    if( PAIR64 ) tuMx64PairBody( stage[wv], sInit[wv], sOps[wv], xch[wv >> 1], &pairCtr[wv >> 1], w & 1, w >> 1, jobs.j[k].waveStride >> 1, resi, rs, jobs.j[k] );
    else         tuMx64Body( stage[wv], sInit[wv], sOps[wv], w, resi, rs, jobs.j[k] );
  }
}

__global__ void __launch_bounds__( 256 )
dequantCoreKernel( int maxX, int maxY, int scale, const int16_t* __restrict__ q, size_t qStride, int32_t* __restrict__ coef, int rightShift, int inMax, int32_t trMax )
{
  const int w = maxX + 1, total = w * ( maxY + 1 );
  for( int n = blockIdx.x * blockDim.x + threadIdx.x; n < total; n += gridDim.x * blockDim.x )
  {
    const int y = n / w, x = n - y * w;
    const int c = clip3i( -( inMax + 1 ), inMax, ( int ) q[x + y * qStride] );
    int32_t v;
    if( rightShift > 0 ) v = ( int32_t ) ( ( uint32_t ) ( c * scale ) + ( 1u << ( rightShift - 1 ) ) ) >> rightShift;
    else                 v = ( int32_t ) ( ( uint32_t ) ( c * scale ) << ( -rightShift ) );
    coef[n] = clip3i( -( trMax + 1 ), trMax, v );
  }
}

__global__ void __launch_bounds__( 256 )
needRdoqCoreKernel( const int32_t* __restrict__ coef, size_t num, int quantCoeff, long long offset, int shift, uint8_t* __restrict__ need )
{
  int any = 0;
  for( size_t i = threadIdx.x; i < num; i += blockDim.x ) any |= ( int32_t ) ( ( ( int64_t ) abs( coef[i] ) * quantCoeff + offset ) >> shift ) != 0;
  __shared__ int sAny;
  if( threadIdx.x == 0 ) sAny = 0;
  __syncthreads();
  if( any ) sAny = 1;
  __syncthreads();
  if( threadIdx.x == 0 ) *need = ( uint8_t ) sAny;
}

bool makeGeom( int w, int h, int trHor, int trVer, int bitDepth, bool inverse, TrGeom& g )
{
  if( !isPow2( w ) || !isPow2( h ) || w < 2 || h < 2 || w > 64 || h > 64 ) return false;
  g.w = w; g.h = h; g.log2w = ilog2i( w ); g.log2h = ilog2i( h );
  auto okType = []( int t, int n ) { return t == VVHIP_DCT2 ? true : ( ( t == VVHIP_DCT8 || t == VVHIP_DST7 ) && n >= 4 && n <= 32 ); };
  if( !okType( trHor, w ) || !okType( trVer, h ) ) return false;
  g.skipW = ( trHor != VVHIP_DCT2 && w == 32 ) ? 16 : ( w > 32 ? w - 32 : 0 );
  g.skipH = ( trVer != VVHIP_DCT2 && h == 32 ) ? 16 : ( h > 32 ? h - 32 : 0 );
  if( !inverse ) { g.shift1 = g.log2w + bitDepth + 6 - 15; g.shift2 = g.log2h + 6; if( g.shift1 < 0 ) return false; }
  else           { g.shift1 = 6 + 1; g.shift2 = ( 6 + 15 - 1 ) - bitDepth; if( g.shift2 < 1 ) return false; }
  return true;
}

bool makeQGeom( int w, int h, int bitDepth, QGeom& q )
{
  if( !isPow2( w ) || !isPow2( h ) || w < 1 || h < 1 || w > 64 || h > 64 || w * h < 2 ) return false;
  q.w = w; q.h = h; q.log2w = ilog2i( w ); q.log2h = ilog2i( h ); q.bitDepth = bitDepth;
  int cgw, cgh;
  vvhip_cg_size( q.log2w, q.log2h, &cgw, &cgh );
  q.log2CG = cgw + cgh;
  q.cgIs4x4 = ( q.log2CG == 4 && cgw == 2 ) ? 1 : 0;
  q.numScan = ( w < 32 ? w : 32 ) * ( h < 32 ? h : 32 );
  return true;
}

int rowPitch( int n )
{
  const int ch = n < 8 ? n : 8;
  int pu = n / ch;
  if( pu > 1 && !( pu & 1 ) ) pu++;
  return pu * ch;
}

TuLay makeLayout( const TrGeom& g, int trHor, int trVer )
{
  TuLay y;
  y.pw = rowPitch( g.w ); y.ph = rowPitch( g.h );
  const int area = g.w * g.h;
  int r = g.h * y.pw > g.w * y.ph ? g.h * y.pw : g.w * y.ph;
  if( r < area ) r = area;
  r = ( r + 7 ) & ~7;
  y.r1 = r; y.r2 = 2 * r; y.slot = 2 * r + 2 * area;
  const bool same = g.w == g.h && trHor == trVer;
  y.mTh = 0; y.mTv = same ? 0 : g.w * g.w;
  const int nat = same ? g.w * g.w : g.w * g.w + g.h * g.h;
  y.mThT = nat; y.mTvT = same ? nat : nat + g.w * g.w;
  y.matElems = 2 * nat;
  return y;
}

size_t trSmemBytes( const TuLay& y, int tpb )
{
// ... 110 lines not shown
                       int16_t* d_level, int32_t* d_delta_u, int32_t* d_abs_sum, int32_t* d_last_scan_pos )
{
  if( !ctx ) return VVHIP_E_ARG;
  QGeom q;
  if( n < 0 || !makeQGeom( width, height, bit_depth, q ) ) return vvhip_fail( ctx, VVHIP_E_ARG, "vvhip_quant_batch: unsupported TU %dx%d", width, height );
  if( n == 0 ) return VVHIP_OK;
  const int log2Lpc = teamLog2( q.numScan );
  const long threads = ( long ) n << log2Lpc;
  hipLaunchKernelGGL( quantKernel, dim3( ( unsigned ) ( ( threads + 255 ) / 256 ) ), dim3( 256 ), 0, ctx->stream,
                      d_coef, n, q, log2Lpc, d_qp, 0, 0, 0ll, thr_val, ctx->d_scan + scanOffset( q.log2w, q.log2h ), d_level, d_delta_u, d_abs_sum, d_last_scan_pos );
  VVHIP_LAUNCH_CHECK( ctx );
  return VVHIP_OK;
}

int vvhip_quant_core_lfnst( vvhip_ctx* ctx, const int32_t* d_coef, int width, int height, int quant_coeff, int q_bits, int64_t add, int thr_val, int lfnst_idx,
                            int16_t* d_level, int32_t* d_delta_u, int32_t* d_abs_sum, int32_t* d_last_scan_pos )
{
  if( !ctx ) return VVHIP_E_ARG;
  QGeom q;
  if( !makeQGeom( width, height, 10, q ) || q_bits < 9 || lfnst_idx < 0 ) return vvhip_fail( ctx, VVHIP_E_ARG, "vvhip_quant_core: unsupported TU %dx%d / qBits %d / lfnstIdx %d", width, height, q_bits, lfnst_idx );
  const int log2Lpc = teamLog2( q.numScan );
  hipLaunchKernelGGL( quantKernel, dim3( 1 ), dim3( 256 ), 0, ctx->stream,
                      d_coef, 1, q, log2Lpc, ( const vvhip_tu_qp* ) nullptr, quant_coeff, q_bits, ( long long ) add, thr_val,
                      ctx->d_scan + scanOffset( q.log2w, q.log2h ), d_level, d_delta_u, d_abs_sum, d_last_scan_pos, lfnst_idx > 0 ? 1 : 0 );
  VVHIP_LAUNCH_CHECK( ctx );
  return VVHIP_OK;
}

int vvhip_quant_core( vvhip_ctx* ctx, const int32_t* d_coef, int width, int height, int quant_coeff, int q_bits, int64_t add, int thr_val,
                      int16_t* d_level, int32_t* d_delta_u, int32_t* d_abs_sum, int32_t* d_last_scan_pos )
{
  return vvhip_quant_core_lfnst( ctx, d_coef, width, height, quant_coeff, q_bits, add, thr_val, 0, d_level, d_delta_u, d_abs_sum, d_last_scan_pos );
}

int vvhip_dequant_batch( vvhip_ctx* ctx, const int16_t* d_level, int n, int width, int height, int bit_depth, const vvhip_tu_qp* d_qp, int32_t* d_coef )
{
  if( !ctx ) return VVHIP_E_ARG;
  QGeom q;
  if( n < 0 || !makeQGeom( width, height, bit_depth, q ) ) return vvhip_fail( ctx, VVHIP_E_ARG, "vvhip_dequant_batch: unsupported TU %dx%d", width, height );
  if( n == 0 ) return VVHIP_OK;
  const long total = ( long ) n * width * height;
  long blocks = ( total + 255 ) / 256; if( blocks > 8192 ) blocks = 8192;
  hipLaunchKernelGGL( dequantKernel, dim3( ( unsigned ) blocks ), dim3( 256 ), 0, ctx->stream, d_level, total, q, d_qp, d_coef );
  VVHIP_LAUNCH_CHECK( ctx );
  return VVHIP_OK;
}

int vvhip_need_rdoq_batch( vvhip_ctx* ctx, const int32_t* d_coef, int n, int width, int height, int bit_depth, const vvhip_tu_qp* d_qp, uint8_t* d_need )
{
  if( !ctx ) return VVHIP_E_ARG;
  QGeom q;
  if( n < 0 || !makeQGeom( width, height, bit_depth, q ) ) return vvhip_fail( ctx, VVHIP_E_ARG, "vvhip_need_rdoq_batch: unsupported TU %dx%d", width, height );
  if( n == 0 ) return VVHIP_OK;
  const int log2Lpc = teamLog2( width * ( height < 32 ? height : 32 ) );
  const long threads = ( long ) n << log2Lpc;
  hipLaunchKernelGGL( needRdoqKernel, dim3( ( unsigned ) ( ( threads + 255 ) / 256 ) ), dim3( 256 ), 0, ctx->stream, d_coef, n, q, log2Lpc, d_qp, d_need );
  VVHIP_LAUNCH_CHECK( ctx );
  return VVHIP_OK;
}

int vvhip_dequant_core( vvhip_ctx* ctx, int max_x, int max_y, int scale, const int16_t* d_level, size_t level_stride, int32_t* d_coef,
                        int right_shift, int input_maximum, int32_t transform_maximum )
{
  if( !ctx ) return VVHIP_E_ARG;
  if( max_x < 0 || max_y < 0 || max_x > 127 || max_y > 127 ) return vvhip_fail( ctx, VVHIP_E_ARG, "vvhip_dequant_core: bad block" );
  const int total = ( max_x + 1 ) * ( max_y + 1 );
  hipLaunchKernelGGL( dequantCoreKernel, dim3( ( total + 255 ) / 256 ), dim3( 256 ), 0, ctx->stream, max_x, max_y, scale, d_level, level_stride, d_coef,
                      right_shift, input_maximum, transform_maximum );
  VVHIP_LAUNCH_CHECK( ctx );
  return VVHIP_OK;
}

static int tuRdoMulti( vvhip_ctx* ctx, const int16_t* d_resi, int resi_stride, const int32_t* strides, int bit_depth, const vvhip_tu_job* jobs, int n_jobs );

int vvhip_tu_rdo_multi( vvhip_ctx* ctx, const int16_t* d_resi, int resi_stride, int bit_depth, const vvhip_tu_job* jobs, int n_jobs )
{
  return tuRdoMulti( ctx, d_resi, resi_stride, nullptr, bit_depth, jobs, n_jobs );
}

int vvhip_tu_set_sparse_outputs( vvhip_ctx* ctx, int on )
{
  if( !ctx ) return VVHIP_E_ARG;
  ctx->tuSparse = on != 0;
  return VVHIP_OK;
}

int vvhip_tu_rdo_multi_strided( vvhip_ctx* ctx, const int16_t* d_resi, const int32_t* resi_strides_host, int bit_depth, const vvhip_tu_job* jobs, int n_jobs )
{
  if( !ctx ) return VVHIP_E_ARG;
  if( n_jobs && !resi_strides_host ) return vvhip_fail( ctx, VVHIP_E_ARG, "vvhip_tu_rdo_multi_strided: no strides" );
  return tuRdoMulti( ctx, d_resi, 0, resi_strides_host, bit_depth, jobs, n_jobs );
}

static int tuRdoMulti( vvhip_ctx* ctx, const int16_t* d_resi, int resi_stride, const int32_t* strides, int bit_depth, const vvhip_tu_job* jobs, int n_jobs )
{
  if( !ctx ) return VVHIP_E_ARG;
  if( n_jobs < 0 || ( n_jobs && !jobs ) ) return vvhip_fail( ctx, VVHIP_E_ARG, "vvhip_tu_rdo_multi: bad job table" );
  auto mergeable = []( const vvhip_tu_job& j ) { return j.n > 0 && j.width == j.height && ( j.width == 8 || j.width == 16 || j.width == 32 ||
                                                        ( tuKernelForm() == 0 && ( j.width == 4 || ( j.width == 64 && j.tr_hor == VVHIP_DCT2 && j.tr_ver == VVHIP_DCT2 ) ) ) ); };
  int order[64], nm = 0;
  std::vector<TuGenJob> gen;
  for( int i = 0; i < n_jobs; i++ )
  {
    if( jobs[i].n < 0 ) return vvhip_fail( ctx, VVHIP_E_ARG, "vvhip_tu_rdo_multi: job %d has n < 0", i );
    if( mergeable( jobs[i] ) && nm < 64 && !getenv( "VVHIP_TU_GENERIC" ) && ( !strides || tuKernelForm() == 0 ) ) order[nm++] = i;
    else if( jobs[i].n > 0 )
    {
      static const bool separate = getenv( "VVHIP_TU_GENERIC_SEPARATE" ) != nullptr;
      const vvhip_tu_job& jb = jobs[i];
      const bool rowForm = jb.width == jb.height && ( jb.width == 8 || jb.width == 16 || jb.width == 32 );
      if( separate || rowForm || gen.size() >= 64 )
      {
        const int rc = vvhip_tu_rdo_batch( ctx, d_resi, strides ? strides[i] : resi_stride, jb.d_resi_off, jb.n, jb.width, jb.height, jb.tr_hor, jb.tr_ver, bit_depth,
                                           jb.d_qp, jb.thr_val, jb.d_level, jb.d_rec_resi, jb.d_stats );
        if( rc ) return rc;
        continue;
      }
      TuGenJob g; memset( &g, 0, sizeof( g ) );
      if( !makeGeom( jb.width, jb.height, jb.tr_hor, jb.tr_ver, bit_depth, false, g.gf ) || !makeGeom( jb.width, jb.height, jb.tr_hor, jb.tr_ver, bit_depth, true, g.gi ) || !makeQGeom( jb.width, jb.height, bit_depth, g.q ) )
        return vvhip_fail( ctx, VVHIP_E_ARG, "vvhip_tu_rdo_multi: unsupported %dx%d types (%d,%d) bitDepth %d", jb.width, jb.height, jb.tr_hor, jb.tr_ver, bit_depth );
      g.y = makeLayout( g.gf, jb.tr_hor, jb.tr_ver );
      const int area = jb.width * jb.height;
      g.tpb = area >= 1024 ? 1 : 1024 / area;
      g.resiStride = strides ? strides[i] : resi_stride; g.n = jb.n; g.thrVal = jb.thr_val;
      g.resiOff = jb.d_resi_off; g.matH = ctx->d_trMat + trMatOffset( jb.tr_hor, g.gf.log2w ); g.matV = ctx->d_trMat + trMatOffset( jb.tr_ver, g.gf.log2h );
      g.scan = ctx->d_scan + scanOffset( g.q.log2w, g.q.log2h ); g.qps = jb.d_qp; g.level = jb.d_level; g.rec = jb.d_rec_resi; g.stats = jb.d_stats;
      gen.push_back( g );
    }
  }
  if( !gen.empty() )
  {
    std::stable_sort( gen.begin(), gen.end(), []( const TuGenJob& a, const TuGenJob& b ) { return a.gf.w * a.gf.h > b.gf.w * b.gf.h; } );
    size_t smem = 0; int blocks = 0;
    for( TuGenJob& g : gen ) { g.blockStart = blocks; blocks += ( g.n + g.tpb - 1 ) / g.tpb; smem = std::max( smem, trSmemBytes( g.y, g.tpb ) ); }
    const size_t bytes = gen.size() * sizeof( TuGenJob );
    if( ctx->tuGenBytes < bytes )
    {
      if( ctx->d_tuGen ) { VVHIP_CHECK_HIP( ctx, hipStreamSynchronize( ctx->stream ) ); ( void ) hipFree( ctx->d_tuGen ); ctx->d_tuGen = nullptr; ctx->tuGenBytes = 0; }
      VVHIP_CHECK_HIP( ctx, hipMalloc( &ctx->d_tuGen, 64 * sizeof( TuGenJob ) ) );
      ctx->tuGenBytes = 64 * sizeof( TuGenJob ); ctx->tuGenLast.clear();
    }
    if( ctx->tuGenStream != ctx->stream )
    {
      const bool wait = !ctx->tuGenLast.empty() && ctx->tuGenEventRecorded;
      ctx->tuGenLast.clear(); ctx->tuGenStream = ctx->stream;
      if( wait ) VVHIP_CHECK_HIP( ctx, hipStreamWaitEvent( ctx->stream, ctx->tuGenEvent, 0 ) );
    }
    if( ctx->tuGenLast.size() != bytes || memcmp( ctx->tuGenLast.data(), gen.data(), bytes ) != 0 )
    {
      ctx->tuGenLast.assign( reinterpret_cast<const unsigned char*>( gen.data() ), reinterpret_cast<const unsigned char*>( gen.data() ) + bytes );
      VVHIP_CHECK_HIP( ctx, hipMemcpyAsync( ctx->d_tuGen, ctx->tuGenLast.data(), bytes, hipMemcpyHostToDevice, ctx->stream ) );
    }
    if( smem > 64 * 1024 ) VVHIP_CHECK_HIP( ctx, hipFuncSetAttribute( ( const void* ) tuRdoGenMultiKernel, hipFuncAttributeMaxDynamicSharedMemorySize, ( int ) smem ) );
    hipLaunchKernelGGL( tuRdoGenMultiKernel, dim3( ( unsigned ) blocks ), dim3( 256 ), smem, ctx->stream, d_resi, static_cast<const TuGenJob*>( ctx->d_tuGen ), ( int ) gen.size(), tuPhaseLimit() );
    VVHIP_LAUNCH_CHECK( ctx );
    if( !ctx->tuGenEvent ) VVHIP_CHECK_HIP( ctx, hipEventCreateWithFlags( &ctx->tuGenEvent, hipEventDisableTiming ) );
    VVHIP_CHECK_HIP( ctx, hipEventRecord( ctx->tuGenEvent, ctx->stream ) );
    ctx->tuGenEventRecorded = true;
  }
  const bool mx = tuKernelForm() == 0;
  const int groupMax = mx ? 8 : 4;
  auto isExtra = [&]( int i ) { return jobs[order[i]].width == 4 || jobs[order[i]].width == 64; };
  auto tilesOf = [&]( int i ) { const vvhip_tu_job& jb = jobs[order[i]]; const int tpt = jb.width == 64 ? 1 : ( 32 / jb.width ) * ( 32 / jb.width ); return ( long ) ( jb.n + tpt - 1 ) / tpt; };
  long allTiles = 0;
  for( int i = 0; i < nm; i++ ) allTiles += tilesOf( i );
  static const long oneLaunchTiles = getenv( "VVHIP_TU_ONE_LAUNCH_TILES" ) ? atol( getenv( "VVHIP_TU_ONE_LAUNCH_TILES" ) ) : 65536;
  static const long repeat1Tiles = getenv( "VVHIP_TU_REPEAT1_TILES" ) ? atol( getenv( "VVHIP_TU_REPEAT1_TILES" ) ) : 16384;
  const bool oneLaunch = mx && nm <= groupMax && allTiles <= oneLaunchTiles;
  static const long smallFirstTiles = getenv( "VVHIP_TU_SMALL_FIRST" ) ? atol( getenv( "VVHIP_TU_SMALL_FIRST" ) ) : 256;
  auto isShort = [&]( int i ) { return oneLaunch && tilesOf( i ) < smallFirstTiles; };
  auto before = [&]( int a, int b ) { const bool ea = isExtra( a ), eb = isExtra( b ), sa = isShort( a ), sb = isShort( b );
                                      return ( !oneLaunch && ea != eb ) ? !ea : ( sa != sb ? sa : jobs[order[a]].width > jobs[order[b]].width ); };
  for( int a = 1; a < nm; a++ ) for( int b = a; b > 0 && before( b, b - 1 ); b-- ) { const int t = order[b]; order[b] = order[b - 1]; order[b - 1] = t; }
  int nRegular = 0;
  while( !oneLaunch && nRegular < nm && !isExtra( nRegular ) ) nRegular++;
  for( int first = 0, next = 0; first < nm; first = next )
  {
    next = first + groupMax;
    if( !oneLaunch && first < nRegular && next > nRegular ) next = nRegular;
    const int groupEnd = next < nm ? next : nm;

    TuMultiJobs mj; mj.nJobs = 0;
    TuRowArgs rowArgs[8];
    int nJobs = 0;
    long blocks = 0, groupTiles = 0;
    for( int i = first; i < groupEnd; i++ ) groupTiles += tilesOf( i );
    static const long residentEnv = getenv( "VVHIP_TU_RESIDENT_WAVES" ) ? atol( getenv( "VVHIP_TU_RESIDENT_WAVES" ) ) : 0;
    const long residentWaves = residentEnv ? residentEnv : 8192;
    int budget = 0;
    static const bool pair64 = getenv( "VVHIP_TU_PAIR64" ) && atoi( getenv( "VVHIP_TU_PAIR64" ) ) == 1;
    auto wavesPer = [&]( int i ) { return ( jobs[order[i]].width == 64 && pair64 ) ? 2 : 1; };
    auto repeatOf = [&]( int i ) { const int work = jobs[order[i]].width == 64 ? ( pair64 ? 2 : 4 ) : 1; const int r = budget / work; return r < 1 ? 1 : r; };
    if( mx && groupTiles <= repeat1Tiles * 4 )
    {
      for( budget = 1; budget < 8; budget++ )
      {
        long waves = 0;
        for( int i = first; i < groupEnd; i++ ) waves += wavesPer( i ) * ( ( tilesOf( i ) + repeatOf( i ) - 1 ) / repeatOf( i ) );
        if( waves <= residentWaves ) break;
      }
    }
    for( int i = first; i < groupEnd; i++ )
    {
      const vvhip_tu_job& jb = jobs[order[i]];
      TuRowArgs& ra = rowArgs[nJobs];
      if( !makeGeom( jb.width, jb.height, jb.tr_hor, jb.tr_ver, bit_depth, false, ra.gf ) || !makeGeom( jb.width, jb.height, jb.tr_hor, jb.tr_ver, bit_depth, true, ra.gi ) ||
          !makeQGeom( jb.width, jb.height, bit_depth, ra.q ) )
        return vvhip_fail( ctx, VVHIP_E_ARG, "vvhip_tu_rdo_multi: unsupported %dx%d types (%d,%d) bitDepth %d", jb.width, jb.height, jb.tr_hor, jb.tr_ver, bit_depth );
      ra.resiOff = jb.d_resi_off; ra.n = jb.n;
      ra.matH = ctx->d_trMat + trMatOffset( jb.tr_hor, ra.gf.log2w ); ra.matV = ctx->d_trMat + trMatOffset( jb.tr_ver, ra.gf.log2h );
      ra.scan = ctx->d_scan + scanOffset( ra.q.log2w, ra.q.log2h );
      ra.qps = jb.d_qp; ra.thrVal = jb.thr_val; ra.level = jb.d_level; ra.rec = jb.d_rec_resi; ra.stats = jb.d_stats; ra.phaseLimit = tuPhaseLimit();
      if( !mx )
      {
        const int tpb = 256 / ( jb.width * ( jb.width == 8 ? 1 : 2 ) );
        mj.blockStart[nJobs] = ( int ) blocks; mj.size[nJobs] = jb.width;
        const int groups = ( jb.n + tpb - 1 ) / tpb;
        ra.groupStride = ( groups + tuRepeat() - 1 ) / tuRepeat();
        blocks += ra.groupStride;
        mj.j[nJobs] = ra;
      }
      nJobs++;
    }
    if( mx )
    {
      TuMxJobs xj; xj.nJobs = nJobs; xj.pair64 = pair64 ? 1 : 0;
      long waves = 0;
      for( int i = 0; i < nJobs; i++ )
      {
        const vvhip_tu_job& jb = jobs[order[first + i]];
        const TuRowArgs& ra = rowArgs[i];
        TuMxArgs& xa = xj.j[i];
        const int z = ra.gf.log2w - 2, tpt = jb.width == 64 ? 1 : ( 32 / jb.width ) * ( 32 / jb.width );
        xa.resiOff = jb.d_resi_off; xa.n = jb.n;
        xa.shF1 = ra.gf.shift1; xa.shF2 = ra.gf.shift2; xa.shI1 = ra.gi.shift1; xa.shI2 = ra.gi.shift2; xa.skipW = ra.gf.skipW; xa.skipH = ra.gf.skipH;
        xa.q = ra.q;
        xa.opH = ctx->d_tuMx + jb.tr_hor * 4 + z; xa.opV = ctx->d_tuMx + jb.tr_ver * 4 + z; xa.pos = ctx->d_tuMxPos + z * 64 * 16;
        if( jb.width == 64 ) { xa.opH = reinterpret_cast<const VvhipTuMxOps*>( ctx->d_tuMx64 ); xa.opV = xa.opH; xa.pos = nullptr; }
        xa.qps = jb.d_qp; xa.thrVal = jb.thr_val; xa.level = jb.d_level; xa.rec = jb.d_rec_resi; xa.stats = jb.d_stats;
        xa.tiles = ( jb.n + tpt - 1 ) / tpt; xa.phaseLimit = tuPhaseLimit() | ( ctx->tuSparse ? 0x100 : 0 );
        const int repeat = budget ? repeatOf( first + i ) : tuRepeat();
        xa.waveStride = wavesPer( first + i ) * ( ( xa.tiles + repeat - 1 ) / repeat );
        xa.resiStride = strides ? strides[order[first + i]] : 0;
        if( wavesPer( first + i ) == 2 ) waves = ( waves + 1 ) & ~1l;
        xj.waveStart[i] = ( int ) waves; xj.size[i] = jb.width;
        waves += xa.waveStride;
      }
      for( int i = nJobs; i < 8; i++ ) { xj.waveStart[i] = 0x7fffffff; xj.size[i] = 0; }
      bool any4 = false;
      for( int i = 0; i < xj.nJobs; i++ ) any4 |= xj.size[i] == 4 || xj.size[i] == 64;
      bool any64 = false;
      for( int i = 0; i < xj.nJobs; i++ ) any64 |= xj.size[i] == 64;
      const char* wg1Env = getenv( "VVHIP_TU_WG1" );
      const int wpb = ( ( !wg1Env || atoi( wg1Env ) != 0 ) && !( any64 && pair64 ) ) ? 1 : 4;
      const dim3 grid( ( unsigned ) ( ( waves + wpb - 1 ) / wpb ) );
      static const int ldsPad = getenv( "VVHIP_TU_LDS_PAD" ) ? atoi( getenv( "VVHIP_TU_LDS_PAD" ) ) : 0;
      static bool padSet = false;
      if( ldsPad > 0 && !padSet )
      {
        padSet = true;
        ( void ) hipFuncSetAttribute( ( const void* ) tuMxMultiKernel<0, 4>, hipFuncAttributeMaxDynamicSharedMemorySize, ldsPad );
        ( void ) hipFuncSetAttribute( ( const void* ) tuMxMultiKernel<1, 4>, hipFuncAttributeMaxDynamicSharedMemorySize, ldsPad );
        ( void ) hipFuncSetAttribute( ( const void* ) tuMxMultiKernel<2, 4>, hipFuncAttributeMaxDynamicSharedMemorySize, ldsPad );
        ( void ) hipFuncSetAttribute( ( const void* ) tuMxMultiKernel<3, 4>, hipFuncAttributeMaxDynamicSharedMemorySize, ldsPad );
        ( void ) hipFuncSetAttribute( ( const void* ) tuMxMultiKernel<0, 1>, hipFuncAttributeMaxDynamicSharedMemorySize, ldsPad );
        ( void ) hipFuncSetAttribute( ( const void* ) tuMxMultiKernel<1, 1>, hipFuncAttributeMaxDynamicSharedMemorySize, ldsPad );
        ( void ) hipFuncSetAttribute( ( const void* ) tuMxMultiKernel<2, 1>, hipFuncAttributeMaxDynamicSharedMemorySize, ldsPad );
      }
      if( any64 && pair64 ) hipLaunchKernelGGL( ( tuMxMultiKernel<3, 4> ), grid, dim3( 256 ), ldsPad, ctx->stream, d_resi, resi_stride, xj );
      else if( wpb == 1 )
      {
        if( any64 )     hipLaunchKernelGGL( ( tuMxMultiKernel<2, 1> ), grid, dim3( 64 ), ldsPad, ctx->stream, d_resi, resi_stride, xj );
        else if( any4 ) hipLaunchKernelGGL( ( tuMxMultiKernel<1, 1> ), grid, dim3( 64 ), ldsPad, ctx->stream, d_resi, resi_stride, xj );
        else            hipLaunchKernelGGL( ( tuMxMultiKernel<0, 1> ), grid, dim3( 64 ), ldsPad, ctx->stream, d_resi, resi_stride, xj );
      }
      else if( any64 ) hipLaunchKernelGGL( ( tuMxMultiKernel<2, 4> ), grid, dim3( 256 ), ldsPad, ctx->stream, d_resi, resi_stride, xj );
      else if( any4 ) hipLaunchKernelGGL( ( tuMxMultiKernel<1, 4> ), grid, dim3( 256 ), ldsPad, ctx->stream, d_resi, resi_stride, xj );
      else            hipLaunchKernelGGL( ( tuMxMultiKernel<0, 4> ), grid, dim3( 256 ), ldsPad, ctx->stream, d_resi, resi_stride, xj );
    }
    else
    {
      mj.nJobs = nJobs;
      for( int i = nJobs; i < 4; i++ ) { mj.blockStart[i] = 0x7fffffff; mj.size[i] = 0; }
      hipLaunchKernelGGL( tuRdoRowMultiKernel, dim3( ( unsigned ) blocks ), dim3( 256 ), 0, ctx->stream, d_resi, resi_stride, mj );
    }
    VVHIP_LAUNCH_CHECK( ctx );
  }
  return VVHIP_OK;
}

static bool trSizeOk( int n ) { return n == 4 || n == 8 || n == 16 || n == 32 || n == 64; }

int vvhip_fast_fwd_core( vvhip_ctx* ctx, int tr_size, const int16_t* d_tc, const int32_t* d_src, int32_t* d_dst, unsigned line, unsigned reduced_line, unsigned cutoff, int shift )
{
  if( !ctx ) return VVHIP_E_ARG;
  if( !trSizeOk( tr_size ) || !d_tc || !d_src || !d_dst || reduced_line > line || cutoff > ( unsigned ) tr_size || line > 64 || shift < 1 || shift > 31 )
    return vvhip_fail( ctx, VVHIP_E_ARG, "vvhip_fast_fwd_core: trSize %d line %u/%u cutoff %u shift %d", tr_size, reduced_line, line, cutoff, shift );
  const unsigned total = reduced_line * cutoff;
  if( !total ) return VVHIP_OK;
  hipLaunchKernelGGL( fastFwdCoreKernel, dim3( ( total + 255 ) / 256 ), dim3( 256 ), 0, ctx->stream, tr_size, d_tc, d_src, d_dst, line, reduced_line, cutoff, shift );
  VVHIP_LAUNCH_CHECK( ctx );
  return VVHIP_OK;
}

int vvhip_fast_inv_core( vvhip_ctx* ctx, int tr_size, const int16_t* d_it, const int32_t* d_src, int32_t* d_dst, unsigned lines, unsigned reduced_lines, unsigned rows )
{
  if( !ctx ) return VVHIP_E_ARG;
  if( !trSizeOk( tr_size ) || !d_it || !d_src || !d_dst || reduced_lines > lines || rows > ( unsigned ) tr_size || lines > 64 )
    return vvhip_fail( ctx, VVHIP_E_ARG, "vvhip_fast_inv_core: trSize %d lines %u/%u rows %u", tr_size, reduced_lines, lines, rows );
  const unsigned total = reduced_lines * tr_size;
  if( !total ) return VVHIP_OK;
  hipLaunchKernelGGL( fastInvCoreKernel, dim3( ( total + 255 ) / 256 ), dim3( 256 ), 0, ctx->stream, tr_size, d_it, d_src, d_dst, lines, reduced_lines, rows );
  VVHIP_LAUNCH_CHECK( ctx );
  return VVHIP_OK;
}

int vvhip_round_clip( vvhip_ctx* ctx, int32_t* d_dst, unsigned width, unsigned height, unsigned stride, int32_t out_min, int32_t out_max, int32_t round, int32_t shift )
{
  if( !ctx ) return VVHIP_E_ARG;
  if( !d_dst || width > stride || shift < 0 || shift > 31 || ( uint64_t ) width * height > ( 1u << 24 ) ) return vvhip_fail( ctx, VVHIP_E_ARG, "vvhip_round_clip: bad arguments" );
  if( !( width * height ) ) return VVHIP_OK;
  hipLaunchKernelGGL( roundClipKernel, dim3( ( width * height + 255 ) / 256 ), dim3( 256 ), 0, ctx->stream, d_dst, width, height, stride, out_min, out_max, round, shift );
  VVHIP_LAUNCH_CHECK( ctx );
  return VVHIP_OK;
}

int vvhip_cpy_resi( vvhip_ctx* ctx, const int32_t* d_src, int16_t* d_dst, ptrdiff_t stride, unsigned width, unsigned height )
{
  if( !ctx ) return VVHIP_E_ARG;
  if( !d_src || !d_dst || ( uint64_t ) width * height > ( 1u << 24 ) ) return vvhip_fail( ctx, VVHIP_E_ARG, "vvhip_cpy_resi: bad arguments" );
  if( !( width * height ) ) return VVHIP_OK;
  hipLaunchKernelGGL( cpyResiKernel, dim3( ( width * height + 255 ) / 256 ), dim3( 256 ), 0, ctx->stream, d_src, d_dst, stride, width, height );
  VVHIP_LAUNCH_CHECK( ctx );
  return VVHIP_OK;
}

int vvhip_cpy_coeff( vvhip_ctx* ctx, const int16_t* d_src, ptrdiff_t stride, int32_t* d_dst, unsigned width, unsigned height )
{
  if( !ctx ) return VVHIP_E_ARG;
  if( !d_src || !d_dst || ( uint64_t ) width * height > ( 1u << 24 ) ) return vvhip_fail( ctx, VVHIP_E_ARG, "vvhip_cpy_coeff: bad arguments" );
  if( !( width * height ) ) return VVHIP_OK;
  hipLaunchKernelGGL( cpyCoeffKernel, dim3( ( width * height + 255 ) / 256 ), dim3( 256 ), 0, ctx->stream, d_src, stride, d_dst, width, height );
  VVHIP_LAUNCH_CHECK( ctx );
  return VVHIP_OK;
}

int vvhip_need_rdoq_core( vvhip_ctx* ctx, const int32_t* d_coef, size_t num_coeff, int quant_coeff, int64_t offset, int shift, uint8_t* d_need )
{
  if( !ctx ) return VVHIP_E_ARG;
  hipLaunchKernelGGL( needRdoqCoreKernel, dim3( 1 ), dim3( 256 ), 0, ctx->stream, d_coef, num_coeff, quant_coeff, ( long long ) offset, shift, d_need );
  VVHIP_LAUNCH_CHECK( ctx );
  return VVHIP_OK;
// ... 57 lines not shown
```

### vvenc_amd/hotpath.py

```python
import ctypes as C

import numpy as np
import torch

from .lib import VVHipError, load_library

DF = {"SSE": 0, "SAD": 1, "HAD": 2, "HAD_fast": 3, "HAD_2SAD": 4}
DCT2, DCT8, DST7 = 0, 1, 2

MV_DTYPE = np.dtype([("x", "<i4"), ("y", "<i4"), ("error", "<i4"), ("rmsme", "<i4"), ("overlap", "<f8")])
DMVR_ITEM_DTYPE = np.dtype([("ref0_off", "<i4"), ("ref1_off", "<i4"), ("frac0_x", "<i2"), ("frac0_y", "<i2"), ("frac1_x", "<i2"), ("frac1_y", "<i2")])
DMVR_RESULT_DTYPE = np.dtype([("mvd_x", "<i2"), ("mvd_y", "<i2"), ("pad", "<i4"), ("min_cost", "<u8")])
SUBPEL_DTYPE = np.dtype([("org_off", "<i4"), ("ref_off", "<i4"), ("frac_x", "<i2"), ("frac_y", "<i2")])
PRED_ITEM_DTYPE = np.dtype([("dst_off", "<i4"), ("org_off", "<i4"), ("ref_off", "<i4", (2,)), ("frac", "<i2", (2, 2)), ("width", "<i2"), ("height", "<i2"),
                            ("ref_plane", "i1", (2,)), ("chroma", "u1"), ("alt_hpel", "u1")])
PRED_EXT_DTYPE = np.dtype([("flags", "u1"), ("pad_dx", "i1", (2,)), ("pad_dy", "i1", (2,)), ("rsv", "u1", (3,))])
PRED_EXT_BDOF, PRED_EXT_DMVR_PAD = 1, 2
PRED_BLEND_DTYPE = np.dtype([("mode", "u1"), ("param", "u1"), ("rsv", "u1", (2,))])
PRED_BLEND_DEFAULT, PRED_BLEND_BCW, PRED_BLEND_GEO = 0, 1, 2
PRED_AFFINE_ITEM_DTYPE = np.dtype([("dst_off", "<i4"), ("org_off", "<i4"), ("ref_off", "<i4", (2,)), ("cpmv", "<i4", (2, 3, 2)), ("cu_x", "<i2"), ("cu_y", "<i2"), ("cu_w", "<i2"),
                                   ("cu_h", "<i2"), ("ref_plane", "i1", (2,)), ("chroma", "u1"), ("six_param", "u1"), ("prof", "u1"), ("rsv", "u1", (3,))])


def dmvr_pred_items(results, start_mv, pos, ref_planes, strides, dx, dy, bdof=True, chroma_planes=None, chroma_strides=None):
# ... 511 lines not shown
        self._ck(self.L.vvhip_pred_affine_batch(self.ctx, C.cast(tab, C.c_void_p), len(planes), it.ctypes.data_as(C.c_void_p) if it.size else None, int(it.size),
                                                int(pic_w), int(pic_h), int(ctu), bit_depth, _ptr(pred), pred_stride,
                                                org.buf_ptr if org is not None else None, org.stride if org is not None else 0, _ptr(resi)))
        return pred

    def subpel_dist_batch(self, func, org, ref, d_items, n, w, h, bit_depth=10, filter_mode=0, use_alt_hpel=False, out=None):
        if out is None:
            out = torch.empty(n, dtype=torch.int64, device=self.device)
        self._ck(self.L.vvhip_subpel_dist_batch(self.ctx, DF[func] if isinstance(func, str) else func, org.buf_ptr, org.stride, ref.buf_ptr, ref.stride,
                                                w, h, bit_depth, filter_mode, int(use_alt_hpel), _ptr(d_items), n, _ptr(out)))
        return out

    def subpel_refine_batch(self, func, org, ref, d_bases, n_blocks, offsets, w, h, bit_depth=10, filter_mode=0, use_alt_hpel=False, out=None):
        offs = np.ascontiguousarray(offsets, np.int16).reshape(-1, 2)
        if out is None:
            out = torch.empty(n_blocks * offs.shape[0], dtype=torch.int64, device=self.device)
        self._ck(self.L.vvhip_subpel_refine_batch(self.ctx, DF[func] if isinstance(func, str) else func, org.buf_ptr, org.stride, ref.buf_ptr, ref.stride, w, h, bit_depth,
                                                  filter_mode, int(use_alt_hpel), _ptr(d_bases), n_blocks, offs.ctypes.data_as(C.c_void_p), offs.shape[0], _ptr(out)))
        return out

    def extend_border(self, plane):
        self._ck(self.L.vvhip_extend_border(self.ctx, plane.buf_ptr, plane.stride, plane.width, plane.height, plane.pad))

    def mctf_subsample(self, src, pad=128):
        dst = Plane(self.device, src.width // 2, src.height // 2, pad)
        self._ck(self.L.vvhip_mctf_subsample(self.ctx, src.buf_ptr, src.stride, src.width, src.height, dst.buf_ptr, dst.stride, pad))
        return dst

    def mctf_error_batch(self, org, buf, d_items, n, w, h, tap4, bit_depth=10):
        out = torch.empty(n, dtype=torch.int32, device=self.device)
        self._ck(self.L.vvhip_mctf_error_batch(self.ctx, org.buf_ptr, org.stride, buf.buf_ptr, buf.stride, w, h, int(tap4), bit_depth, _ptr(d_items), n, _ptr(out)))
        return out

    def mctf_calc_var_batch(self, org, d_off, n, w, h):
        out = torch.empty(n, dtype=torch.int64, device=self.device)
        self._ck(self.L.vvhip_mctf_calc_var_batch(self.ctx, org.buf_ptr, org.stride, w, h, _ptr(d_off), n, _ptr(out)))
        return out

    def new_mv_field(self, w, h):
        t = torch.empty((h * w, MV_DTYPE.itemsize), dtype=torch.uint8, device=self.device)
        self._ck(self.L.vvhip_mctf_init_mvs(self.ctx, _ptr(t), w * h))
        return t

    def mctf_me_level(self, org, buf, block_size, prev, prev_dims, factor, double_res, mvs, mvs_dims, search_pattern=2, low_res=1, bit_depth=10, unit=16):
        pw, ph = prev_dims if prev is not None else (0, 0)
        self._ck(self.L.vvhip_mctf_me_level(self.ctx, org.buf_ptr, org.stride, buf.buf_ptr, buf.stride, org.width, org.height, block_size,
                                            _ptr(prev), pw, ph, factor, int(double_res), search_pattern, int(low_res), bit_depth, unit,
                                            _ptr(mvs), mvs_dims[0], mvs_dims[1]))
        return mvs

    def mctf_motion_estimation(self, cur, refs, bit_depth=10, unit=16, speed=4, add_level=None, out=None, wait=True):
        if add_level is None:
            add_level = cur.width >= 1920
        ow, oh = (cur.width + unit - 1) // unit, (cur.height + unit - 1) // unit
        if out is None:
            out = [torch.empty((ow * oh, MV_DTYPE.itemsize), dtype=torch.uint8, device=self.device) for _ in refs]
        ref_ptrs = (C.c_void_p * len(refs))(*[r.buf_ptr.value for r in refs])
        out_ptrs = (C.c_void_p * len(refs))(*[o.data_ptr() for o in out])
        for r in refs:
            assert (r.width, r.height, r.stride, r.pad) == (cur.width, cur.height, cur.stride, cur.pad)
        fn = self.L.vvhip_mctf_motion_estimation if wait else self.L.vvhip_mctf_motion_estimation_async
        self._ck(fn(self.ctx, cur.buf_ptr, ref_ptrs, len(refs), cur.stride, cur.width, cur.height, cur.pad, bit_depth, unit, speed, int(bool(add_level)), out_ptrs))
        return out, (ow, oh)

    def mctf_set_stats(self, on):
        self._ck(self.L.vvhip_mctf_set_stats(self.ctx, int(bool(on))))

    def quant_core(self, coef, quant_coeff, q_bits, add, thr_val=8, lfnst_idx=0):
        coef = np.ascontiguousarray(coef, np.int32)
        h, w = coef.shape
        d_c = self.to_device(coef.reshape(-1))
        d_l = torch.full((h * w,), 0x7777, dtype=torch.int16, device=self.device)
        d_u = torch.zeros(h * w, dtype=torch.int32, device=self.device)
        d_s = torch.zeros(2, dtype=torch.int32, device=self.device)
        self._ck(self.L.vvhip_quant_core_lfnst(self.ctx, _ptr(d_c), w, h, quant_coeff, q_bits, add, thr_val, int(lfnst_idx), _ptr(d_l), _ptr(d_u), C.c_void_p(d_s.data_ptr()),
                                               C.c_void_p(d_s.data_ptr() + 4)))
        torch.cuda.synchronize()
        sv = d_s.cpu().numpy()
        return d_l.cpu().numpy().reshape(h, w), d_u.cpu().numpy(), int(sv[0]), int(sv[1])

    def tu_set_sparse_outputs(self, on):
        self._ck(self.L.vvhip_tu_set_sparse_outputs(self.ctx, int(bool(on))))

    def mctf_set_timing(self, on):
        self._ck(self.L.vvhip_mctf_set_timing(self.ctx, int(bool(on))))

    def mctf_last_times(self):
        a = (C.c_float * 5)()
        self._ck(self.L.vvhip_mctf_last_times(self.ctx, a))
        return tuple(float(x) for x in a)

    def mctf_get_stats(self):
        a = np.zeros(24, np.uint64)
        self._ck(self.L.vvhip_mctf_get_stats(self.ctx, a.ctypes.data_as(C.c_void_p)))
        keys = ("int", "int_bytes", "frac", "frac_bytes", "grid", "grid_window_bytes", "ring", "ring_window_bytes")
        return {ph: {k: int(a[8 * i + j]) for j, k in enumerate(keys)} for i, ph in enumerate(("search", "neighbour", "sweep"))}

    @staticmethod
    def mv_to_numpy(t, dims):
        return t.cpu().numpy().view(MV_DTYPE).reshape(dims[1], dims[0])
```

### vvenc_amd/lib.py

```python
import ctypes as C
import os

HERE = os.path.dirname(os.path.abspath(__file__))
LIB_PATH = os.environ.get("VVHIP_LIB") or os.path.join(HERE, "libvvenc_hip.so")


class VVHipError(RuntimeError):
    pass


vp, i32, u64p, sz = C.c_void_p, C.c_int, C.c_void_p, C.c_size_t

PROTOTYPES = {
    "vvhip_create": (i32, [C.POINTER(vp), i32]),
    "vvhip_destroy": (None, [vp]),
    "vvhip_last_error": (C.c_char_p, [vp]),
    "vvhip_set_stream": (i32, [vp, vp]),
    "vvhip_use_own_stream": (i32, [vp]),
    "vvhip_get_stream": (vp, [vp]),
    "vvhip_sync": (i32, [vp]),
    "vvhip_sync_all_devices": (i32, [vp]),
    "vvhip_set_blocking_sync": (i32, [vp, i32]),
    "vvhip_malloc": (i32, [vp, C.POINTER(vp), sz]),
    "vvhip_free": (i32, [vp, vp]),
# ... 8 lines not shown
    "vvhip_host_free": (i32, [vp, vp]),
    "vvhip_event_create": (i32, [vp, C.POINTER(vp)]),
    "vvhip_event_record": (i32, [vp, vp]),
    "vvhip_event_wait": (i32, [vp, vp]),
    "vvhip_event_destroy": (i32, [vp, vp]),
    "vvhip_device_count": (i32, []),
    "vvhip_get_device": (i32, [vp]),
    "vvhip_make_current": (i32, [vp]),
    "vvhip_copy_peer": (i32, [vp, vp, vp, vp, sz]),
    "vvhip_version": (C.c_char_p, []),
    "vvhip_dist_batch": (i32, [vp, i32, vp, i32, vp, i32, i32, i32, i32, i32, vp, i32, vp]),
    "vvhip_dist_multi": (i32, [vp, i32, vp, i32, vp, i32, i32, vp, i32]),
    "vvhip_dist_multi_func": (i32, [vp, vp, i32, vp, i32, i32, vp, i32]),
    "vvhip_tiled8_elems": (sz, [i32, i32]),
    "vvhip_plane_tile8": (i32, [vp, vp, i32, i32, vp]),
    "vvhip_plane_shift1": (i32, [vp, vp, C.c_size_t, vp]),
    "vvhip_planes_derive": (i32, [vp, vp, i32, i32, vp, vp, i32, i32, vp, vp]),
    "vvhip_dist_multi_func_tiled": (i32, [vp, vp, i32, vp, i32, vp, i32, vp, i32]),
    "vvhip_sad_mask_batch": (i32, [vp, vp, i32, vp, i32, vp, i32, i32, i32, i32, i32, i32, i32, vp, vp, i32, vp]),
    "vvhip_fix_weighted_sse_batch": (i32, [vp, vp, i32, vp, i32, i32, i32, i32, vp, vp, i32, vp]),
    "vvhip_sad_x5_batch": (i32, [vp, vp, i32, vp, i32, i32, i32, i32, i32, vp, i32, vp]),
    "vvhip_sad_surface": (i32, [vp, vp, i32, vp, i32, i32, i32, i32, i32, i32, vp, vp, i32, vp]),
    "vvhip_fwd_transform_batch": (i32, [vp, vp, i32, vp, i32, i32, i32, i32, i32, i32, vp]),
    "vvhip_inv_transform_batch": (i32, [vp, vp, i32, i32, i32, i32, i32, i32, vp, i32, vp]),
    "vvhip_quant_batch": (i32, [vp, vp, i32, i32, i32, i32, vp, i32, vp, vp, vp, vp]),
    "vvhip_dequant_batch": (i32, [vp, vp, i32, i32, i32, i32, vp, vp]),
    "vvhip_need_rdoq_batch": (i32, [vp, vp, i32, i32, i32, i32, vp, vp]),
    "vvhip_dequant_core": (i32, [vp, i32, i32, i32, vp, sz, vp, i32, i32, i32]),
    "vvhip_quant_core": (i32, [vp, vp, i32, i32, i32, i32, C.c_int64, i32, vp, vp, vp, vp]),
    "vvhip_quant_core_lfnst": (i32, [vp, vp, i32, i32, i32, i32, C.c_int64, i32, i32, vp, vp, vp, vp]),
    "vvhip_need_rdoq_core": (i32, [vp, vp, sz, i32, C.c_int64, i32, vp]),
    "vvhip_tu_rdo_batch": (i32, [vp, vp, i32, vp, i32, i32, i32, i32, i32, i32, vp, i32, vp, vp, vp]),
    "vvhip_tu_rdo_multi": (i32, [vp, vp, i32, i32, vp, i32]),
    "vvhip_tu_rdo_multi_strided": (i32, [vp, vp, vp, i32, vp, i32]),
    "vvhip_me_plan_create": (i32, [vp, vp, i32, vp, i32, vp, i32, vp, i32, i32, i32, C.POINTER(vp)]),
    "vvhip_me_plan_create_lists": (i32, [vp, vp, i32, i32, C.POINTER(vp)]),
    "vvhip_me_plan_destroy": (None, [vp, vp]),
    "vvhip_me_plan_run": (i32, [vp, vp, vp, i32, vp, vp, vp]),
    "vvhip_me_plan_run_parts": (i32, [vp, vp, vp, i32, vp, vp, vp, i32]),
    "vvhip_me_plan_info": (i32, [vp, vp, vp, vp, vp]),
    "vvhip_me_plan_set_timing": (i32, [vp, vp, i32]),
    "vvhip_me_plan_last_times": (i32, [vp, vp, vp]),
    "vvhip_fast_fwd_core": (i32, [vp, i32, vp, vp, vp, C.c_uint, C.c_uint, C.c_uint, i32]),
    "vvhip_fast_inv_core": (i32, [vp, i32, vp, vp, vp, C.c_uint, C.c_uint, C.c_uint]),
    "vvhip_round_clip": (i32, [vp, vp, C.c_uint, C.c_uint, C.c_uint, i32, i32, i32, i32]),
    "vvhip_cpy_resi": (i32, [vp, vp, vp, C.c_ssize_t, C.c_uint, C.c_uint]),
    "vvhip_cpy_coeff": (i32, [vp, vp, C.c_ssize_t, vp, C.c_uint, C.c_uint]),
    "vvhip_if_filter": (i32, [vp, i32, i32, i32, i32, i32, vp, i32, vp, i32, i32, i32, vp]),
    "vvhip_if_copy": (i32, [vp, i32, i32, i32, vp, i32, vp, i32, i32, i32, i32]),
    "vvhip_interp_luma_batch": (i32, [vp, vp, i32, vp, i32, i32, i32, i32, i32, i32, i32, vp]),
    "vvhip_interp_chroma_batch": (i32, [vp, vp, i32, vp, i32, i32, i32, i32, i32, vp]),
    "vvhip_pred_inter_batch": (i32, [vp, vp, i32, vp, i32, i32, vp, i32, vp, i32, vp]),
    "vvhip_pred_inter_batch_ex": (i32, [vp, vp, i32, vp, vp, i32, i32, vp, i32, vp, i32, vp]),
    "vvhip_pred_inter_batch_blend": (i32, [vp, vp, i32, vp, vp, vp, i32, i32, vp, i32, vp, i32, vp]),
    "vvhip_pred_affine_batch": (i32, [vp, vp, i32, vp, i32, i32, i32, i32, i32, vp, i32, vp, i32, vp]),
    "vvhip_subpel_dist_batch": (i32, [vp, i32, vp, i32, vp, i32, i32, i32, i32, i32, i32, vp, i32, vp]),
    "vvhip_mctf_apply_plane": (i32, [vp, vp, i32, i32, i32, i32, i32, i32, i32, i32, i32, vp, i32, vp, i32, vp, C.c_double, C.c_double, vp, i32]),
    "vvhip_mctf_filter_params": (i32, [i32, i32, C.c_double, i32, vp, vp]),
    "vvhip_dmvr_refine_batch": (i32, [vp, vp, i32, vp, i32, vp, i32, i32, i32, i32, vp]),
    "vvhip_alf_classify": (i32, [vp, vp, i32, i32, i32, i32, i32, i32, vp]),
    "vvhip_ccalf_stats_plane": (i32, [vp, vp, i32, vp, i32, vp, i32, i32, i32, i32, i32, i32, i32, i32, i32, vp, vp]),
    "vvhip_alf_stats_plane_units": (i32, [vp, vp, i32, vp, i32, i32, i32, i32, i32, i32, vp, i32, i32, vp, vp]),
    "vvhip_alf_stats_plane": (i32, [vp, vp, i32, vp, i32, i32, i32, i32, i32, vp, i32, i32, vp, vp]),
    "vvhip_graph_begin": (i32, [vp]),
    "vvhip_graph_end": (i32, [vp, vp]),
    "vvhip_graph_launch": (i32, [vp, vp]),
    "vvhip_graph_destroy": (None, [vp]),
    "vvhip_alf_filter_plane": (i32, [vp, vp, C.c_ssize_t, vp, C.c_ssize_t, i32, i32, i32, i32, i32, vp, vp, vp, vp, i32, i32]),
    "vvhip_ccalf_filter_plane": (i32, [vp, vp, C.c_ssize_t, vp, C.c_ssize_t, i32, i32, i32, i32, i32, i32, vp, vp, i32, i32]),
    "vvhip_subpel_refine_batch": (i32, [vp, i32, vp, i32, vp, i32, i32, i32, i32, i32, i32, vp, i32, vp, i32, vp]),
    "vvhip_get_tr_matrix_host": (i32, [i32, i32, vp]),
    "vvhip_get_scan_order_host": (i32, [i32, i32, vp]),
    "vvhip_get_me_tap_tables_host": (i32, [i32, vp]),
    "vvhip_get_geo_weights_host": (i32, [i32, i32, i32, i32, vp]),
    "vvhip_mctf_error_batch": (i32, [vp, vp, i32, vp, i32, i32, i32, i32, i32, vp, i32, vp]),
    "vvhip_mctf_calc_var_batch": (i32, [vp, vp, i32, i32, i32, vp, i32, vp]),
    "vvhip_mctf_subsample": (i32, [vp, vp, i32, i32, i32, vp, i32, i32]),
    "vvhip_extend_border": (i32, [vp, vp, i32, i32, i32, i32]),
    "vvhip_mctf_init_mvs": (i32, [vp, vp, i32]),
    "vvhip_mctf_me_level": (i32, [vp, vp, i32, vp, i32, i32, i32, i32, vp, i32, i32, i32, i32, i32, i32, i32, i32, vp, i32, i32]),
    "vvhip_mctf_motion_estimation": (i32, [vp, vp, vp, i32, i32, i32, i32, i32, i32, i32, i32, i32, vp]),
    "vvhip_mctf_motion_estimation_async": (i32, [vp, vp, vp, i32, i32, i32, i32, i32, i32, i32, i32, i32, vp]),
    "vvhip_tu_set_sparse_outputs": (i32, [vp, i32]),
    "vvhip_mctf_set_stats": (i32, [vp, i32]),
    "vvhip_mctf_get_stats": (i32, [vp, vp]),
    "vvhip_mctf_set_timing": (i32, [vp, i32]),
    "vvhip_mctf_last_times": (i32, [vp, vp]),
}

_lib = None


def load_library(path=None):
    global _lib
    if _lib is not None and path is None:
        return _lib
    p = path or LIB_PATH
    try:
        import torch
    except ImportError:
        pass
    if not os.path.exists(p):
        raise VVHipError("%s not found - build it with `make -C vvenc_amd/csrc` (hipcc --offload-arch=gfx950); "
                         "vvenc_amd has no CPU fallback" % p)
    lib = C.CDLL(p)
    for name, (res, args) in PROTOTYPES.items():
        fn = getattr(lib, name)
        fn.restype = res
        fn.argtypes = args
    if path is None:
        _lib = lib
    return lib
```

### vvenc_amd/replay.py

```python
import ctypes as C
import os

import numpy as np
import torch

from . import recorded as R
from .hotpath import DF, HotPath, Plane, STATS_DTYPE, DMVR_ITEM_DTYPE, DMVR_RESULT_DTYPE

ME_INT_JOB = np.dtype([("org_off", "<i4"), ("ref_off", "<i4"), ("width", "<i2"), ("height", "<i2"), ("org_plane", "u1"), ("ref_plane", "u1"), ("sub_shift", "u1"), ("reserved", "u1"),
                       ("min_dx", "<i2"), ("min_dy", "<i2"), ("win_w", "<i2"), ("win_h", "<i2"), ("first_cand", "<i4"), ("n_cand", "<i4")])
ME_CAND = np.dtype([("dx", "<i2"), ("dy", "<i2")])
ME_STAGE_JOB = np.dtype([("org_off", "<i4"), ("ref_off", "<i4"), ("width", "<i2"), ("height", "<i2"), ("org_plane", "u1"), ("ref_plane", "u1"), ("i_frac", "u1"), ("filter_mode", "u1"),
                         ("alt_hpel", "u1"), ("func", "u1"), ("base_qx", "i1"), ("base_qy", "i1"), ("mask", "<u2"), ("reserved", "<u2")])
ME_ITEM = np.dtype([("org_off", "<i4"), ("cur_off", "<i4"), ("org_plane", "u1"), ("cur_plane", "u1"), ("func", "u1"), ("sub_shift", "u1"), ("width", "<i2"), ("height", "<i2")])
ME_MASK_ITEM = np.dtype([("org_off", "<i4"), ("cur_off", "<i4"), ("mask_off", "<i4"), ("org_plane", "u1"), ("cur_plane", "u1"), ("mask_plane", "u1"), ("sub_shift", "u1"),
                         ("width", "<i2"), ("height", "<i2"), ("reserved", "<i4")])
assert ME_INT_JOB.itemsize == 32 and ME_STAGE_JOB.itemsize == 24 and ME_ITEM.itemsize == 16 and ME_MASK_ITEM.itemsize == 24


class MePlane(C.Structure):
    _fields_ = [("d_base", C.c_void_p), ("stride", C.c_int32), ("reserved", C.c_int32)]


FAMILY_TO_FUNC = {"SSE": DF["SSE"], "SAD": DF["SAD"], "HAD": DF["HAD"], "HAD_fast": DF["HAD_fast"], "HAD_2SAD": DF["HAD_2SAD"]}
# ... 283 lines not shown
            pool_sel = op == self.pool_index
            uniq["ME_int"] = plane_union([ref_r, org_r]) + 2 * _covered_1d(self.pool.size, jobs["org_off"][pool_sel], (w_ * h_)[pool_sel]) + 32 * jobs.size + 12 * pc.size
        else:
            uniq["ME_int"] = 0
        if sj.size:
            taps = np.where(sj["filter_mode"] == 2, 4, np.where(sj["filter_mode"] == 1, 6, 8)).astype(np.int64)
            rx, ry = xy(sj["ref_off"], st_n[sj["ref_plane"]])
            w_, h_ = sj["width"].astype(np.int64), sj["height"].astype(np.int64)
            ref_r = (sj["ref_plane"].astype(np.int64), rx - taps // 2, ry - taps // 2, rx + w_ + taps // 2 + 1, ry + h_ + taps // 2 + 1)
            op = sj["org_plane"].astype(np.int64)
            ox_, oy_ = xy(sj["org_off"], st_n[np.minimum(op, self.n_pic_planes)])
            pool_sel = op == self.pool_index
            uniq["ME_stage"] = plane_union([ref_r, (op, ox_, oy_, ox_ + w_, oy_ + h_)]) + 2 * _covered_1d(self.pool.size, sj["org_off"][pool_sel], (w_ * h_)[pool_sel]) + (24 + 72) * sj.size
        else:
            uniq["ME_stage"] = 0
        rects, pool_off, pool_len = [], [], []
        for arr, fields in ((self.items, (("org_plane", "org_off"), ("cur_plane", "cur_off"))), (mi, (("org_plane", "org_off"), ("cur_plane", "cur_off"), ("mask_plane", "mask_off")))):
            if not arr.size:
                continue
            w_, h_ = arr["width"].astype(np.int64), arr["height"].astype(np.int64)
            for fp, fo in fields:
                op = arr[fp].astype(np.int64)
                x_, y_ = xy(arr[fo], st_n[np.minimum(op, self.n_pic_planes)])
                rects.append((op, x_, y_, x_ + w_, y_ + h_))
                sel_p = op == self.pool_index
                pool_off.append(arr[fo][sel_p].astype(np.int64))
                pool_len.append((w_ * h_)[sel_p])
        uniq["ME_item"] = (plane_union(rects) + 2 * _covered_1d(self.pool.size, np.concatenate(pool_off), np.concatenate(pool_len)) if rects else 0) + 24 * self.items.size + 32 * mi.size
        uniq["TU"] = (2 * _covered_1d(self.pool.size, np.concatenate([g["off"].astype(np.int64) for g in self.tu_groups]), np.concatenate([np.full(g["n"], g["w"] * g["h"], np.int64) for g in self.tu_groups]))
                      + int(sum(g["n"] * (4 * g["w"] * g["h"] + 24 + 8) for g in self.tu_groups))) if self.tu_groups else 0
        du = 0
        for g in self.dmvr_groups:
            it = g["items"]
            r0 = (np.full(g["n"], g["r0"], np.int64),) + tuple(v for v in (lambda x_, y_: (x_ - 2, y_ - 2, x_ + g["dx"] + 3, y_ + g["dy"] + 3))(*xy(it["ref0_off"], strides[g["r0"]])))
            r1 = (np.full(g["n"], g["r1"], np.int64),) + tuple(v for v in (lambda x_, y_: (x_ - 2, y_ - 2, x_ + g["dx"] + 3, y_ + g["dy"] + 3))(*xy(it["ref1_off"], strides[g["r1"]])))
            du += plane_union([r0, r1]) + g["n"] * (16 + 16)
        uniq["DMVR"] = du
        self.unique_bytes_by_kernel = {k: int(v) for k, v in uniq.items()}
        self.alg_bytes_tu = int(sum(g["n"] * (6 * g["w"] * g["h"] + 24) for g in self.tu_groups))
        self.alg_bytes_dmvr = int(sum(g["n"] * (2 * 2 * (g["dx"] + 5) * (g["dy"] + 5) + 16) for g in self.dmvr_groups))


class RecordedWorkload:

    def __init__(self, hp: HotPath, pic, max_window=16, bit_depth=10, unique_bytes=True):
        lists = pic if isinstance(pic, RecordedLists) else RecordedLists(pic, bit_depth, unique_bytes)
        self.hp, self.lists, self.pic, self.bit_depth = hp, lists, lists.pic, lists.bit_depth
        dev = hp.device
        for k in ("n_pic_planes", "pool_index", "n_planes", "mask_items", "mask_expected", "dropped", "nothing_dropped", "int_jobs", "plan_cands", "cand_expected", "cand_index", "stage_jobs", "stage_index", "stage_expected", "stage_evaluated", "items",
                  "item_expected", "items_dropped", "tu_coefficients", "pairs", "alg_bytes_me", "alg_bytes_int_all_candidates", "alg_bytes_int_per_position", "alg_bytes_int_window", "int_positions_distinct", "alg_bytes_by_kernel", "alg_bytes_tu", "alg_bytes_dmvr", "unique_bytes_by_kernel"):
            setattr(self, k, getattr(lists, k))
        self.planes = []
        for hpl in lists.planes:
            pl = Plane(dev, hpl.width, hpl.height, hpl.pad)
            assert pl.stride == hpl.stride
            pl.storage = torch.from_numpy(hpl.storage).to(dev)
            self.planes.append(pl)
        self.pool = torch.from_numpy(lists.pool).to(dev)
        tab = (MePlane * 16)()
        for i, pl in enumerate(self.planes):
            tab[i] = MePlane(pl.storage.data_ptr() + 2 * pl.origin, pl.stride, 0)
        tab[self.pool_index] = MePlane(self.pool.data_ptr(), 0, 0)
        self.plane_table = tab
        self.plan = hp.me_plan_create(self.int_jobs, self.plan_cands, self.stage_jobs, self.items, bit_depth, max_window, mask_items=self.mask_items)
        self.cand_cost = torch.zeros(max(1, self.plan_cands.size), dtype=torch.int64, device=dev)
        self.stage_cost = torch.zeros(max(1, 9 * self.stage_jobs.size), dtype=torch.int64, device=dev)
        self.item_cost = torch.zeros(max(1, self.items.size + self.mask_items.size), dtype=torch.int64, device=dev)
        self.me_info = hp.me_plan_info(self.plan)
        self._me_call = hp.bound("vvhip_me_plan_run", self.plan, C.cast(self.plane_table, C.c_void_p), self.n_planes, C.c_void_p(self.cand_cost.data_ptr()),
                                 C.c_void_p(self.stage_cost.data_ptr()), C.c_void_p(self.item_cost.data_ptr()))

        self.tu_groups, tu_jobs, strides_l = [], [], []
        for g in lists.tu_groups:
            n, w, h = g["n"], g["w"], g["h"]
            d = dict(g, d_off=hp.to_device(g["off"]), d_qp=hp.to_device(g["qf"]), level=torch.empty(n * w * h, dtype=torch.int16, device=dev),
                     rec=torch.empty(n * w * h, dtype=torch.int16, device=dev), stats=torch.empty((n, 24), dtype=torch.uint8, device=dev))
            self.tu_groups.append(d)
            tu_jobs.append((w, h, g["tr_hor"], g["tr_ver"], n, 8, d["d_off"], d["d_qp"], d["level"], d["rec"], d["stats"]))
            strides_l.append(w)
        self.tu_table = hp.make_tu_jobs(tu_jobs) if tu_jobs else None
        self.tu_sparse = os.environ.get("VVHIP_TU_SPARSE", "1") != "0"
        hp.tu_set_sparse_outputs(self.tu_sparse)
        self.tu_strides = (C.c_int32 * max(1, len(strides_l)))(*strides_l)
        self._tu_call = hp.bound("vvhip_tu_rdo_multi_strided", C.c_void_p(self.pool.data_ptr()), C.cast(self.tu_strides, C.c_void_p), bit_depth, self.tu_table[0], self.tu_table[1]) if tu_jobs else None
        self.dmvr_groups = [dict(g, d_items=hp.to_device(g["items"]), out=torch.zeros((g["n"], 16), dtype=torch.uint8, device=dev)) for g in lists.dmvr_groups]
        self._dmvr_calls = [hp.bound("vvhip_dmvr_refine_batch", self.planes[g["r0"]].buf_ptr, self.planes[g["r0"]].stride, self.planes[g["r1"]].buf_ptr, self.planes[g["r1"]].stride,
                                     C.c_void_p(g["d_items"].data_ptr()), g["n"], g["dx"], g["dy"], bit_depth, C.c_void_p(g["out"].data_ptr())) for g in self.dmvr_groups]

    def bind_lanes(self, lanes):
        args = (self.plan, C.cast(self.plane_table, C.c_void_p), self.n_planes, C.c_void_p(self.cand_cost.data_ptr()), C.c_void_p(self.stage_cost.data_ptr()), C.c_void_p(self.item_cost.data_ptr()))
        if len(lanes) >= 5:
            me = [lanes[0].bound("vvhip_me_plan_run_parts", *args, 1), lanes[1].bound("vvhip_me_plan_run_parts", *args, 2), lanes[2].bound("vvhip_me_plan_run_parts", *args, 4)]
            hp1, hp2 = lanes[3], lanes[4]
        else:
            me = [lanes[0].bound("vvhip_me_plan_run", *args)]
            hp1, hp2 = lanes[1], lanes[2]
        hp1.tu_set_sparse_outputs(self.tu_sparse)
        tus = [hp1.bound("vvhip_tu_rdo_multi_strided", C.c_void_p(self.pool.data_ptr()), C.cast(self.tu_strides, C.c_void_p), self.bit_depth, self.tu_table[0], self.tu_table[1])] if self.tu_table else []
        dm = [hp2.bound("vvhip_dmvr_refine_batch", self.planes[g["r0"]].buf_ptr, self.planes[g["r0"]].stride, self.planes[g["r1"]].buf_ptr, self.planes[g["r1"]].stride,
                        C.c_void_p(g["d_items"].data_ptr()), g["n"], g["dx"], g["dy"], self.bit_depth, C.c_void_p(g["out"].data_ptr())) for g in self.dmvr_groups]
        skip = set(filter(None, os.environ.get("VVHIP_BENCH_SKIP_LANES", "").split(",")))
        if skip:
            if len(me) == 3:
                me = [c for c, name in zip(me, ("stage", "int", "item")) if name not in skip]
            tus = [] if "tu" in skip else tus
            dm = [] if "dmvr" in skip else dm
        self._lane_calls = [c for c in me + tus + dm if c is not None]
        return self._lane_calls

    def run_lanes(self):
        for c in self._lane_calls:
            c()

    def run_me(self):
        self._me_call()

    def update_tu_alg_bytes(self):
        from .hotpath import STATS_DTYPE
        torch.cuda.synchronize()
        tot = zero_tus = zero_area = area = 0
        for g in self.tu_groups:
            wh = g["w"] * g["h"]
            nz = int((g["stats"].cpu().numpy().view(STATS_DTYPE).reshape(-1)["abs_sum"] == 0).sum()) if self.tu_sparse else 0
            tot += nz * (2 * wh + 24) + (g["n"] - nz) * (6 * wh + 24)
            zero_tus += nz
            zero_area += nz * wh
            area += g["n"] * wh
        self.alg_bytes_tu = int(tot)
        self.tu_zero_share = {"tus": zero_tus, "area_share": round(zero_area / area, 4) if area else None}
        return self.alg_bytes_tu

    def run_tu(self):
        if self._tu_call is not None:
            self._tu_call()

    def run_dmvr(self):
        for c in self._dmvr_calls:
            c()

    def run(self, timers=None):
        for cls, fn in (("ME", self.run_me), ("TU", self.run_tu), ("DMVR", self.run_dmvr)):
            if timers is not None:
                timers.start(cls)
            fn()
            if timers is not None:
                timers.stop(cls)

    @property
    def distinct_positions(self):
        return self.int_positions_distinct

    @property
    def class_launches(self):
        return {"ME": 1, "TU": max(1, len({(g["w"] in (4, 64)) for g in self.tu_groups})), "DMVR": max(1, len(self.dmvr_groups))}

    def check_against_recording(self):
        torch.cuda.synchronize()
        out = {}
        got = self.cand_cost.cpu().numpy().view(np.uint64)[:self.plan_cands.size]
        out["integer_candidates"] = (int(self.plan_cands.size), int((got != self.cand_expected).sum()))
        gs = self.stage_cost.cpu().numpy().view(np.uint64)[:9 * self.stage_jobs.size].reshape(-1, 9)
        out["subpel_positions"] = (int(self.stage_evaluated.sum()), int(((gs != self.stage_expected) & self.stage_evaluated).sum()))
        gi = self.item_cost.cpu().numpy().view(np.uint64)[:self.items.size + self.mask_items.size]
        out["table_calls"] = (int(self.items.size), int((gi[:self.items.size] != self.item_expected).sum()))
        if self.mask_items.size:
            out["masked_sad_calls"] = (int(self.mask_items.size), int((gi[self.items.size:] != self.mask_expected).sum()))
        dm = self.pic.dmvr
        n_d = bad_d = 0
        for g in self.dmvr_groups:
            res = g["out"].cpu().numpy().view(DMVR_RESULT_DTYPE).reshape(-1)
            e = dm[g["index"]]
            bad_d += int(((res["mvd_x"] != e["mvdX"]) | (res["mvd_y"] != e["mvdY"]) | (res["min_cost"] != e["minCost"])).sum())
            n_d += g["n"]
        out["dmvr_subblocks"] = (n_d, bad_d)
        return out
```

Baseline: 14960 frames/s.

## Split TU RDO into a zero-screening launch and a compacted nonzero-tile launch

Adds a two-pass mode for the fused TU transform/quant kernel. The first launch handles all-zero tiles on its fast path and appends each nonzero tile index to a device list via atomics. The second launch processes only the listed tiles, with wave counts capped, so waves that would sit idle on all-zero tiles stop holding the heavy RDO path back. In exchange it adds an extra launch, atomic list traffic, double-buffered counters reset by the next call, and a fallback when the stream is being captured.

```diff
diff --git a/include/vvenc_hip.h b/include/vvenc_hip.h
--- a/include/vvenc_hip.h
+++ b/include/vvenc_hip.h
@@ -167,6 +167,8 @@
 
 VVHIP_API int vvhip_tu_set_sparse_outputs( vvhip_ctx* ctx, int on );
 
+VVHIP_API int vvhip_tu_set_two_pass( vvhip_ctx* ctx, int mode );
+
 VVHIP_API int vvhip_fast_fwd_core( vvhip_ctx* ctx, int tr_size, const int16_t* d_tc, const int32_t* d_src, int32_t* d_dst,
                                    unsigned line, unsigned reduced_line, unsigned cutoff, int shift );
 VVHIP_API int vvhip_fast_inv_core( vvhip_ctx* ctx, int tr_size, const int16_t* d_it, const int32_t* d_src, int32_t* d_dst,
diff --git a/vvenc_amd/csrc/common.h b/vvenc_amd/csrc/common.h
--- a/vvenc_amd/csrc/common.h
+++ b/vvenc_amd/csrc/common.h
@@ -30,6 +30,11 @@
   size_t       tuGenBytes = 0;
   std::vector<unsigned char> tuGenLast;
   bool         tuSparse   = false;
+  int          tuTwoPass  = 1;
+  int*         d_tuList   = nullptr;
+  size_t       tuListInts = 0;
+  unsigned     tuListCalls = 0;
+  hipStream_t  tuListStream = nullptr;
   hipStream_t  tuGenStream = nullptr;
   hipEvent_t   tuGenEvent  = nullptr;
   bool         tuGenEventRecorded = false;
diff --git a/vvenc_amd/csrc/ctx.hip b/vvenc_amd/csrc/ctx.hip
--- a/vvenc_amd/csrc/ctx.hip
+++ b/vvenc_amd/csrc/ctx.hip
@@ -232,6 +232,7 @@
   if( ctx->d_scratch ) ( void ) hipFree( ctx->d_scratch );
   if( ctx->d_subpel ) ( void ) hipFree( ctx->d_subpel );
   if( ctx->d_tuGen ) ( void ) hipFree( ctx->d_tuGen );
+  if( ctx->d_tuList ) ( void ) hipFree( ctx->d_tuList );
   if( ctx->syncEvent ) ( void ) hipEventDestroy( ctx->syncEvent );
   if( ctx->tuGenEvent ) ( void ) hipEventDestroy( ctx->tuGenEvent );
   for( vvhip_ctx::PredSched& S : ctx->predSched )
diff --git a/vvenc_amd/csrc/trquant.hip b/vvenc_amd/csrc/trquant.hip
--- a/vvenc_amd/csrc/trquant.hip
+++ b/vvenc_amd/csrc/trquant.hip
@@ -814,6 +814,9 @@
 #ifndef TUMX_ZERO_MIN_N
 #define TUMX_ZERO_MIN_N 8
 #endif
+#ifndef TUMX_SCREEN_WAVES
+#define TUMX_SCREEN_WAVES 4
+#endif
 typedef int v4i  __attribute__( ( ext_vector_type( 4 ) ) );
 typedef int v16i __attribute__( ( ext_vector_type( 16 ) ) );
 
@@ -902,13 +905,16 @@
   }
 }
 
-template<int N>
+template<int N, int MODE>
 __device__ __forceinline__ void
-tuMxBody( int16_t* __restrict__ stage, int32_t* __restrict__ sInit, v4i* __restrict__ sOps, const int waveIndex, const int16_t* __restrict__ resi, const int resiStride, const TuMxArgs& A )
+tuMxBody( int16_t* __restrict__ stage, int32_t* __restrict__ sInit, v4i* __restrict__ sOps, const int waveIndex, const int16_t* __restrict__ resi, const int resiStride, const TuMxArgs& A,
+          int* __restrict__ list, int* __restrict__ cnt, const int count )
 {
   constexpr int TPS = 32 / N, TPT = TPS * TPS, R = N >= 16 ? 1 : 16 / N, VPR = 16 / R, G = N == 32 ? 64 : N;
   constexpr int PS = N < 8 ? N : 8, NP = 16 / PS;
   constexpr int LP = 40;
+  constexpr bool LISTED = MODE == 2 && N >= TUMX_ZERO_MIN_N;
+  static_assert( MODE != 1 || N >= TUMX_ZERO_MIN_N, "the screening launch holds only bodies with the all-zero shortcut" );
   struct __attribute__( ( packed, aligned( 2 ) ) ) U16 { u32x4 v; };
   struct __attribute__( ( packed, aligned( 2 ) ) ) U8 { u32x2 v; };
   const int lane = threadIdx.x & 63, h = lane >> 5, c32 = lane & 31;
@@ -946,7 +952,8 @@
     }
   };
   uint32_t xr[8];
-  loadResidual( waveIndex, xr );
+  const int tile0 = LISTED ? __builtin_amdgcn_readfirstlane( list[waveIndex] ) : waveIndex;
+  loadResidual( tile0, xr );
 
   const int rndF1 = A.shF1 > 0 ? 1 << ( A.shF1 - 1 ) : 0, rndF2 = 1 << ( A.shF2 - 1 ), rndI1 = 1 << ( A.shI1 - 1 ), rndI2 = 1 << ( A.shI2 - 1 );
   const bool liveCol = inL < N - A.skipW, liveRow = mxSigma( c32 ) % N < N - A.skipH;
@@ -966,10 +973,12 @@
   WAVE_SYNC();
   if( ( A.phaseLimit & 0xff ) == 1 ) return;
 
-  for( int tile = waveIndex; tile < A.tiles; tile += A.waveStride )
-  {
+  const int itEnd = LISTED ? count : A.tiles;
+  for( int it = waveIndex; it < itEnd; it += A.waveStride )
+  {
+    const int tile = LISTED ? ( it == waveIndex ? tile0 : __builtin_amdgcn_readfirstlane( list[it] ) ) : it;
     v4i aLo, aHi;
-    if( tile != waveIndex ) loadResidual( tile, xr );
+    if( it != waveIndex ) loadResidual( tile, xr );
 #pragma unroll
     for( int g = 0; g < 4; g++ )
     {
@@ -1115,7 +1124,7 @@
       const int tu = tile * TPT + blkL * TPS + blk0 + r; \
       if( A.stats && ( N < 32 || h == 0 ) && inL == r && tu < A.n ) A.stats[tu].sse = t; \
     } }
-    const bool allZero = ( N >= TUMX_ZERO_MIN_N ) && __builtin_amdgcn_ballot_w64( someLevel ) == 0ull;
+    const bool allZero = !LISTED && ( N >= TUMX_ZERO_MIN_N ) && __builtin_amdgcn_ballot_w64( someLevel ) == 0ull;
     uint32_t xr2[8];
 #define TUMX_REREAD() { _Pragma( "unroll" ) for( int c = 0; c < NP; c++ )                                                                \
       {                                                                                                                                 \
@@ -1175,6 +1184,11 @@
 #pragma unroll
       for( int v = 0; v < 16; v++ ) d[v] = 0;
       TUMX_TAIL( false )
+      continue;
+    }
+    if( MODE == 1 )
+    {
+      if( lane == 0 ) { const int slot = atomicAdd( cnt, 1 ); list[slot] = tile; }
       continue;
     }
     uint32_t absSum[R];
@@ -1285,9 +1299,10 @@
 #undef TUMX_TAIL
 }
 
+template<int MODE>
 __device__ __forceinline__ void
 tuMx64Body( int16_t* __restrict__ stage, int32_t* __restrict__ sInit , v4i* __restrict__ sOps , const int waveIndex,
-            const int16_t* __restrict__ resi, const int resiStride, const TuMxArgs& A )
+            const int16_t* __restrict__ resi, const int resiStride, const TuMxArgs& A, int* __restrict__ list, int* __restrict__ cnt, const int count )
 {
   constexpr int LP = 40;
   struct __attribute__( ( packed, aligned( 2 ) ) ) U16 { u32x4 v; };
@@ -1315,8 +1330,10 @@
   }
   WAVE_SYNC();
 
-  for( int tu = waveIndex; tu < A.n; tu += A.waveStride )
-  {
+  const int itEnd = MODE == 2 ? count : A.n;
+  for( int it = waveIndex; it < itEnd; it += A.waveStride )
+  {
+    const int tu = MODE == 2 ? __builtin_amdgcn_readfirstlane( list[it] ) : it;
     const int16_t* src = resi + A.resiOff[tu];
     const vvhip_tu_qp qq = A.qps[tu];
     int d[16];
@@ -1400,7 +1417,7 @@
       if( big < 16 ) last = 15;
       else if( ( big >> 4 ) != ( last >> 4 ) ) last = ( big >> 4 ) * 16 + 15;
     }
-    if( __builtin_amdgcn_ballot_w64( ( ( ( int64_t ) mx * P.scale + P.addQ ) >> P.qBits ) != 0 ) == 0ull )
+    if( MODE != 2 && __builtin_amdgcn_ballot_w64( ( ( ( int64_t ) mx * P.scale + P.addQ ) >> P.qBits ) != 0 ) == 0ull )
     {
       if( A.stats && lane == 0 )
       {
@@ -1442,6 +1459,11 @@
       }
       sse0 = vvhipGroupSum64( sse0, 64, lane );
       if( A.stats && lane == 0 ) A.stats[tu].sse = sse0;
+      continue;
+    }
+    if( MODE == 1 )
+    {
+      if( lane == 0 ) { const int slot = atomicAdd( cnt, 1 ); list[slot] = tu; }
       continue;
     }
     uint32_t sum = 0;
@@ -1768,14 +1790,17 @@
 #undef WAVE_SYNC
 }
 
-struct TuMxJobs { int nJobs; int pair64; int waveStart[8]; int size[8]; TuMxArgs j[8]; };
-
-template<int KIND, int WPB>
-__global__ void __launch_bounds__( 64 * WPB, KIND == 3 ? 2 : 3 )
+struct TuMxJobs { int nJobs; int pair64; int waveStart[8]; int size[8]; TuMxArgs j[8]; int* cnt; int* list; int* cntOther; int listStart[8]; };
+#define TUMX_LIST_COUNTERS 64
+
+template<int KIND, int WPB, int MODE = 0>
+__global__ void __launch_bounds__( 64 * WPB, MODE == 1 ? TUMX_SCREEN_WAVES : ( KIND == 3 ? 2 : 3 ) )
 tuMxMultiKernel( const int16_t* __restrict__ resi, int resiStride, TuMxJobs jobs )
 {
-  constexpr bool WITH4 = KIND >= 1, WITH64 = KIND >= 2, PAIR64 = KIND == 3;
+  constexpr bool WITH4 = KIND >= 1 && MODE != 1, WITH64 = KIND >= 2, PAIR64 = KIND == 3;
   static_assert( WPB == 4 || ( WPB == 1 && !PAIR64 ), "the pair form needs both waves of a pair in one workgroup" );
+  static_assert( MODE == 0 || ( WPB == 1 && !PAIR64 ), "the two-launch form runs one wave per workgroup" );
+  static_assert( MODE != 1 || KIND != 1, "4-point lists are not screened" );
   __shared__ __attribute__( ( aligned( 16 ) ) ) int16_t stage[WPB][32 * 40];
   __shared__ __attribute__( ( aligned( 16 ) ) ) int32_t sInit[WPB][WITH64 ? 96 : 64];
   __shared__ v4i sOps[WPB][PAIR64 ? 512 : ( WITH64 ? 256 : 128 )];
@@ -1784,20 +1809,25 @@
   if( PAIR64 ) { if( threadIdx.x < 2 ) pairCtr[threadIdx.x] = 0; __syncthreads(); }
   const int wv = WPB == 1 ? 0 : __builtin_amdgcn_readfirstlane( ( int ) ( threadIdx.x >> 6 ) );
   const int wave = blockIdx.x * WPB + wv;
+  if( MODE == 2 && wave == 0 ) { static_assert( TUMX_LIST_COUNTERS == 64, "one counter per lane" ); jobs.cntOther[threadIdx.x] = 0; }
   int k = 0;
 #pragma unroll
   for( int i = 1; i < 8; i++ ) if( i < jobs.nJobs && wave >= jobs.waveStart[i] ) k = i;
   const int w = wave - jobs.waveStart[k];
   if( w >= jobs.j[k].waveStride ) return;
+  int count = 0;
+  if( MODE == 2 && ( !WITH4 || jobs.size[k] != 4 ) ) { count = jobs.cnt[k]; if( w >= count ) return; }
+  int* const list = MODE ? jobs.list + jobs.listStart[k] : nullptr;
+  int* const cnt = MODE ? jobs.cnt + k : nullptr;
   const int rs = jobs.j[k].resiStride ? jobs.j[k].resiStride : resiStride;
-  if( jobs.size[k] == 32 )      tuMxBody<32>( stage[wv], sInit[wv], sOps[wv], w, resi, rs, jobs.j[k] );
-  else if( jobs.size[k] == 16 ) tuMxBody<16>( stage[wv], sInit[wv], sOps[wv], w, resi, rs, jobs.j[k] );
-  else if( jobs.size[k] == 8 )  tuMxBody<8>( stage[wv], sInit[wv], sOps[wv], w, resi, rs, jobs.j[k] );
-  else if( WITH4 && jobs.size[k] == 4 )   tuMxBody<4>( stage[wv], sInit[wv], sOps[wv], w, resi, rs, jobs.j[k] );
+  if( jobs.size[k] == 32 )      tuMxBody<32, MODE>( stage[wv], sInit[wv], sOps[wv], w, resi, rs, jobs.j[k], list, cnt, count );
+  else if( jobs.size[k] == 16 ) tuMxBody<16, MODE>( stage[wv], sInit[wv], sOps[wv], w, resi, rs, jobs.j[k], list, cnt, count );
+  else if( jobs.size[k] == 8 )  tuMxBody<8, MODE>( stage[wv], sInit[wv], sOps[wv], w, resi, rs, jobs.j[k], list, cnt, count );
+  else if( WITH4 && jobs.size[k] == 4 )   { if constexpr( WITH4 ) tuMxBody<4, MODE>( stage[wv], sInit[wv], sOps[wv], w, resi, rs, jobs.j[k], list, cnt, count ); }
   else if( WITH64 && jobs.size[k] == 64 )
   {
     if( PAIR64 ) tuMx64PairBody( stage[wv], sInit[wv], sOps[wv], xch[wv >> 1], &pairCtr[wv >> 1], w & 1, w >> 1, jobs.j[k].waveStride >> 1, resi, rs, jobs.j[k] );
-    else         tuMx64Body( stage[wv], sInit[wv], sOps[wv], w, resi, rs, jobs.j[k] );
+    else         tuMx64Body<MODE>( stage[wv], sInit[wv], sOps[wv], w, resi, rs, jobs.j[k], list, cnt, count );
   }
 }
 
@@ -2074,6 +2104,14 @@
 {
   if( !ctx ) return VVHIP_E_ARG;
   ctx->tuSparse = on != 0;
+  return VVHIP_OK;
+}
+
+int vvhip_tu_set_two_pass( vvhip_ctx* ctx, int mode )
+{
+  if( !ctx ) return VVHIP_E_ARG;
+  if( mode != 0 && mode != 1 ) return vvhip_fail( ctx, VVHIP_E_ARG, "vvhip_tu_set_two_pass: mode %d", mode );
+  ctx->tuTwoPass = mode;
   return VVHIP_OK;
 }
 
@@ -2166,6 +2204,9 @@
   for( int a = 1; a < nm; a++ ) for( int b = a; b > 0 && before( b, b - 1 ); b-- ) { const int t = order[b]; order[b] = order[b - 1]; order[b - 1] = t; }
   int nRegular = 0;
   while( !oneLaunch && nRegular < nm && !isExtra( nRegular ) ) nRegular++;
+  bool listReady = false;
+  int listSet = 0, listPairs = 0;
+  long listAt = 0;
   for( int first = 0, next = 0; first < nm; first = next )
   {
     next = first + groupMax;
@@ -2217,6 +2258,8 @@
     if( mx )
     {
       TuMxJobs xj; xj.nJobs = nJobs; xj.pair64 = pair64 ? 1 : 0;
+      xj.cnt = xj.list = xj.cntOther = nullptr;
+      for( int i = 0; i < 8; i++ ) xj.listStart[i] = 0;
       long waves = 0;
       for( int i = 0; i < nJobs; i++ )
       {
@@ -2258,8 +2301,66 @@
         ( void ) hipFuncSetAttribute( ( const void* ) tuMxMultiKernel<0, 1>, hipFuncAttributeMaxDynamicSharedMemorySize, ldsPad );
         ( void ) hipFuncSetAttribute( ( const void* ) tuMxMultiKernel<1, 1>, hipFuncAttributeMaxDynamicSharedMemorySize, ldsPad );
         ( void ) hipFuncSetAttribute( ( const void* ) tuMxMultiKernel<2, 1>, hipFuncAttributeMaxDynamicSharedMemorySize, ldsPad );
-      }
-      if( any64 && pair64 ) hipLaunchKernelGGL( ( tuMxMultiKernel<3, 4> ), grid, dim3( 256 ), ldsPad, ctx->stream, d_resi, resi_stride, xj );
+        ( void ) hipFuncSetAttribute( ( const void* ) tuMxMultiKernel<0, 1, 1>, hipFuncAttributeMaxDynamicSharedMemorySize, ldsPad );
+        ( void ) hipFuncSetAttribute( ( const void* ) tuMxMultiKernel<2, 1, 1>, hipFuncAttributeMaxDynamicSharedMemorySize, ldsPad );
+        ( void ) hipFuncSetAttribute( ( const void* ) tuMxMultiKernel<0, 1, 2>, hipFuncAttributeMaxDynamicSharedMemorySize, ldsPad );
+        ( void ) hipFuncSetAttribute( ( const void* ) tuMxMultiKernel<1, 1, 2>, hipFuncAttributeMaxDynamicSharedMemorySize, ldsPad );
+        ( void ) hipFuncSetAttribute( ( const void* ) tuMxMultiKernel<2, 1, 2>, hipFuncAttributeMaxDynamicSharedMemorySize, ldsPad );
+      }
+      bool twoPass = ctx->tuTwoPass == 1 && wpb == 1 && !( tuPhaseLimit() & 0xff ) && listPairs < TUMX_LIST_COUNTERS / 8;
+      if( twoPass ) { twoPass = false; for( int i = 0; i < xj.nJobs; i++ ) twoPass |= xj.size[i] != 4; }
+      if( twoPass && !listReady )
+      {
+        hipStreamCaptureStatus cap = hipStreamCaptureStatusNone;
+        if( hipStreamIsCapturing( ctx->stream, &cap ) != hipSuccess ) { ( void ) hipGetLastError(); cap = hipStreamCaptureStatusNone; }
+        if( cap != hipStreamCaptureStatusNone ) { twoPass = false; listPairs = TUMX_LIST_COUNTERS / 8; }
+      }
+      if( twoPass && !listReady )
+      {
+        if( ctx->tuListInts < ( size_t ) allTiles )
+        {
+          if( ctx->d_tuList ) { VVHIP_CHECK_HIP( ctx, vvhip_wait_stream( ctx ) ); ( void ) hipFree( ctx->d_tuList ); ctx->d_tuList = nullptr; ctx->tuListInts = 0; }
+          const size_t room = ( size_t ) allTiles + ( size_t ) allTiles / 2 + 1024;
+          VVHIP_CHECK_HIP( ctx, hipMalloc( ( void** ) &ctx->d_tuList, ( 2 * TUMX_LIST_COUNTERS + room ) * sizeof( int ) ) );
+          ctx->tuListInts = room; ctx->tuListCalls = 0; ctx->tuListStream = ctx->stream;
+          VVHIP_CHECK_HIP( ctx, hipMemsetAsync( ctx->d_tuList, 0, 2 * TUMX_LIST_COUNTERS * sizeof( int ), ctx->stream ) );
+        }
+        if( ctx->tuListStream != ctx->stream ) { VVHIP_CHECK_HIP( ctx, hipDeviceSynchronize() ); ctx->tuListStream = ctx->stream; }
+        listSet = ( int ) ( ctx->tuListCalls++ & 1u );
+        listReady = true;
+      }
+      if( twoPass )
+      {
+        const char* lwEnv = getenv( "VVHIP_TU_LONG_WAVES" );
+        const long longCap = lwEnv && atol( lwEnv ) > 0 ? atol( lwEnv ) : 3072;
+        xj.cnt = ctx->d_tuList + listSet * TUMX_LIST_COUNTERS + 8 * listPairs;
+        xj.cntOther = ctx->d_tuList + ( listSet ^ 1 ) * TUMX_LIST_COUNTERS;
+        xj.list = ctx->d_tuList + 2 * TUMX_LIST_COUNTERS + listAt;
+        TuMxJobs sj = xj, lj = xj;
+        long at = 0, waves1 = 0, waves2 = 0;
+        for( int i = 0; i < xj.nJobs; i++ )
+        {
+          sj.listStart[i] = lj.listStart[i] = ( int ) at;
+          at += xj.j[i].tiles;
+          const bool four = xj.size[i] == 4;
+          sj.waveStart[i] = ( int ) waves1; if( four ) sj.j[i].waveStride = 0;
+          waves1 += sj.j[i].waveStride;
+          const long w2 = four ? xj.j[i].waveStride : ( xj.j[i].tiles < longCap ? xj.j[i].tiles : longCap );
+          lj.waveStart[i] = ( int ) waves2; lj.j[i].waveStride = ( int ) w2;
+          waves2 += w2;
+        }
+        listAt += at; listPairs++;
+        const dim3 grid1( ( unsigned ) waves1 ), grid2( ( unsigned ) waves2 );
+        if( any64 ) hipLaunchKernelGGL( ( tuMxMultiKernel<2, 1, 1> ), grid1, dim3( 64 ), ldsPad, ctx->stream, d_resi, resi_stride, sj );
+        else        hipLaunchKernelGGL( ( tuMxMultiKernel<0, 1, 1> ), grid1, dim3( 64 ), ldsPad, ctx->stream, d_resi, resi_stride, sj );
+        VVHIP_LAUNCH_CHECK( ctx );
+        bool has4 = false;
+        for( int i = 0; i < xj.nJobs; i++ ) has4 |= xj.size[i] == 4;
+        if( any64 )     hipLaunchKernelGGL( ( tuMxMultiKernel<2, 1, 2> ), grid2, dim3( 64 ), ldsPad, ctx->stream, d_resi, resi_stride, lj );
+        else if( has4 ) hipLaunchKernelGGL( ( tuMxMultiKernel<1, 1, 2> ), grid2, dim3( 64 ), ldsPad, ctx->stream, d_resi, resi_stride, lj );
+        else            hipLaunchKernelGGL( ( tuMxMultiKernel<0, 1, 2> ), grid2, dim3( 64 ), ldsPad, ctx->stream, d_resi, resi_stride, lj );
+      }
+      else if( any64 && pair64 ) hipLaunchKernelGGL( ( tuMxMultiKernel<3, 4> ), grid, dim3( 256 ), ldsPad, ctx->stream, d_resi, resi_stride, xj );
       else if( wpb == 1 )
       {
         if( any64 )     hipLaunchKernelGGL( ( tuMxMultiKernel<2, 1> ), grid, dim3( 64 ), ldsPad, ctx->stream, d_resi, resi_stride, xj );
diff --git a/vvenc_amd/hotpath.py b/vvenc_amd/hotpath.py
--- a/vvenc_amd/hotpath.py
+++ b/vvenc_amd/hotpath.py
@@ -617,6 +617,9 @@
     def tu_set_sparse_outputs(self, on):
         self._ck(self.L.vvhip_tu_set_sparse_outputs(self.ctx, int(bool(on))))
 
+    def tu_set_two_pass(self, mode):
+        self._ck(self.L.vvhip_tu_set_two_pass(self.ctx, int(mode)))
+
     def mctf_set_timing(self, on):
         self._ck(self.L.vvhip_mctf_set_timing(self.ctx, int(bool(on))))
 
diff --git a/vvenc_amd/lib.py b/vvenc_amd/lib.py
--- a/vvenc_amd/lib.py
+++ b/vvenc_amd/lib.py
@@ -114,6 +114,7 @@
     "vvhip_mctf_motion_estimation": (i32, [vp, vp, vp, i32, i32, i32, i32, i32, i32, i32, i32, i32, vp]),
     "vvhip_mctf_motion_estimation_async": (i32, [vp, vp, vp, i32, i32, i32, i32, i32, i32, i32, i32, i32, vp]),
     "vvhip_tu_set_sparse_outputs": (i32, [vp, i32]),
+    "vvhip_tu_set_two_pass": (i32, [vp, i32]),
     "vvhip_mctf_set_stats": (i32, [vp, i32]),
     "vvhip_mctf_get_stats": (i32, [vp, vp]),
     "vvhip_mctf_set_timing": (i32, [vp, i32]),
diff --git a/vvenc_amd/replay.py b/vvenc_amd/replay.py
--- a/vvenc_amd/replay.py
+++ b/vvenc_amd/replay.py
@@ -389,10 +389,22 @@
         self.tu_sparse = os.environ.get("VVHIP_TU_SPARSE", "1") != "0"
         hp.tu_set_sparse_outputs(self.tu_sparse)
         self.tu_strides = (C.c_int32 * max(1, len(strides_l)))(*strides_l)
-        self._tu_call = hp.bound("vvhip_tu_rdo_multi_strided", C.c_void_p(self.pool.data_ptr()), C.cast(self.tu_strides, C.c_void_p), bit_depth, self.tu_table[0], self.tu_table[1]) if tu_jobs else None
+        self.tu_two_pass = 1 if (self.int_jobs.size or self.stage_jobs.size or self.items.size) else 0
+        if os.environ.get("VVHIP_TU_TWO_PASS", "") in ("0", "1"):
+            self.tu_two_pass = int(os.environ["VVHIP_TU_TWO_PASS"])
+        self._tu_call = self._tu_bound(hp, bit_depth) if tu_jobs else None
         self.dmvr_groups = [dict(g, d_items=hp.to_device(g["items"]), out=torch.zeros((g["n"], 16), dtype=torch.uint8, device=dev)) for g in lists.dmvr_groups]
         self._dmvr_calls = [hp.bound("vvhip_dmvr_refine_batch", self.planes[g["r0"]].buf_ptr, self.planes[g["r0"]].stride, self.planes[g["r1"]].buf_ptr, self.planes[g["r1"]].stride,
                                      C.c_void_p(g["d_items"].data_ptr()), g["n"], g["dx"], g["dy"], bit_depth, C.c_void_p(g["out"].data_ptr())) for g in self.dmvr_groups]
+
+    def _tu_bound(self, hp, bit_depth):
+        mode = hp.bound("vvhip_tu_set_two_pass", self.tu_two_pass)
+        tu = hp.bound("vvhip_tu_rdo_multi_strided", C.c_void_p(self.pool.data_ptr()), C.cast(self.tu_strides, C.c_void_p), bit_depth, self.tu_table[0], self.tu_table[1])
+
+        def call():
+            mode()
+            tu()
+        return call
 
     def bind_lanes(self, lanes):
         args = (self.plan, C.cast(self.plane_table, C.c_void_p), self.n_planes, C.c_void_p(self.cand_cost.data_ptr()), C.c_void_p(self.stage_cost.data_ptr()), C.c_void_p(self.item_cost.data_ptr()))
@@ -403,7 +415,7 @@
             me = [lanes[0].bound("vvhip_me_plan_run", *args)]
             hp1, hp2 = lanes[1], lanes[2]
         hp1.tu_set_sparse_outputs(self.tu_sparse)
-        tus = [hp1.bound("vvhip_tu_rdo_multi_strided", C.c_void_p(self.pool.data_ptr()), C.cast(self.tu_strides, C.c_void_p), self.bit_depth, self.tu_table[0], self.tu_table[1])] if self.tu_table else []
+        tus = [self._tu_bound(hp1, self.bit_depth)] if self.tu_table else []
         dm = [hp2.bound("vvhip_dmvr_refine_batch", self.planes[g["r0"]].buf_ptr, self.planes[g["r0"]].stride, self.planes[g["r1"]].buf_ptr, self.planes[g["r1"]].stride,
                         C.c_void_p(g["d_items"].data_ptr()), g["n"], g["dx"], g["dy"], self.bit_depth, C.c_void_p(g["out"].data_ptr())) for g in self.dmvr_groups]
         skip = set(filter(None, os.environ.get("VVHIP_BENCH_SKIP_LANES", "").split(",")))
```

Result: slower. 12530 frames/s (-16.2%).
